# LDeakin/VkVolume

Measured on AMD Instinct MI355X. Metric: Mray/s, higher is better.
Workload: dtype f32

## Files before the change

### vkvolume_amd/csrc/ray_setup.hpp

```cpp
#pragma once

#include "raymarch_args.hpp"
#include "volume_sampling.hpp"

template <int SKIP, bool FAST>
__device__ __forceinline__ bool ray_setup_impl(const RayMarchArgs &A, uint32_t px, uint32_t py, Ray &R, OrdRange &ord)
{
	R.r = R.g = R.b = R.a = 0.0f;
	R.depth = 0.0f;
	R.n_vol = R.n_dist = R.n_empty = 0;
	R.n_steps = 0, R.i = 0, R.i_min = 0, R.first_hit = 0, R.ul = 0;
	R.fragment = false;
	const int W = A.W, H = A.H, D = A.D;

	const float fx = (float) px + 0.5f, fy = (float) py + 0.5f;
	float       dx = __builtin_fmaf(fy, A.ddy[0], __builtin_fmaf(fx, A.ddx[0], A.dir00[0]));
	float       dy = __builtin_fmaf(fy, A.ddy[1], __builtin_fmaf(fx, A.ddx[1], A.dir00[1]));
	float       dz = __builtin_fmaf(fy, A.ddy[2], __builtin_fmaf(fx, A.ddx[2], A.dir00[2]));
	{
		const float len = __builtin_sqrtf(__builtin_fmaf(dz, dz, __builtin_fmaf(dy, dy, dx * dx)));
		if (FAST)
		{
			ord_both(ord, dx, dy, dz);
			const float r = recip_refined(len);
			dx = div_by(dx, len, r), dy = div_by(dy, len, r), dz = div_by(dz, len, r);
		}
		else
			dx /= len, dy /= len, dz /= len;
	}
	const float ox = A.cam[0], oy = A.cam[1], oz = A.cam[2];
	float       t_near = -INFINITY, t_far = INFINITY;
	bool        miss   = false;
	{
		const float dv[3] = {dx, dy, dz}, ov[3] = {ox, oy, oz};
#pragma unroll
		for (int a = 0; a < 3; ++a)
		{
			if (dv[a] == 0.0f)
			{
				if (ov[a] < 0.0f || ov[a] > 1.0f)
					miss = true;
			}
			else
			{
				float inv;
				if (FAST)
				{
					ord_low(ord, dv[a]);
					inv = recip_exact(dv[a]);
				}
				else
					inv = 1.0f / dv[a];
				const float ta = (0.0f - ov[a]) * inv, tb = (1.0f - ov[a]) * inv;
				t_near = g_max(t_near, g_min(ta, tb));
				t_far  = g_min(t_far, g_max(ta, tb));
			}
		}
	}
	if (miss)
		return false;
	const float Ap = __builtin_fmaf(A.plane_tex[2], oz, __builtin_fmaf(A.plane_tex[1], oy, A.plane_tex[0] * ox)) + A.plane_tex[3];
	const float Bp = __builtin_fmaf(A.plane_tex[2], dz, __builtin_fmaf(A.plane_tex[1], dy, A.plane_tex[0] * dx));
	if (!(Bp > 0.0f))
		return false;
	float t_plane;
	if (FAST)
	{
		ord_both(ord, Bp), ord_both(ord, Ap);
		t_plane = div_by(0.0f - Ap, Bp, recip_refined(Bp));
	}
	else
		t_plane = (0.0f - Ap) / Bp;
	const float t0      = g_max(t_near, t_plane);
	if (!(t0 < t_far))
		return false;
	const float ex = __builtin_fmaf(t0, dx, ox), ey = __builtin_fmaf(t0, dy, oy), ez = __builtin_fmaf(t0, dz, oz);
	R.fragment = true;

	float frag_depth = 0.0f, frag_depth_front = 0.0f, position[4] = {0, 0, 0, 0};
	if (A.depth_attachment)
	{
		const float pm[4] = {ex - 0.5f, ey - 0.5f, ez - 0.5f, 1.0f};
		float       a4[4], b4[4];
		mat4_mul_vec4(A.model, pm, a4);
		mat4_mul_vec4(A.view, a4, b4);
		mat4_mul_vec4(A.proj, b4, position);
		frag_depth       = A.in_depth[R.o];
		frag_depth_front = position[2] / position[3];
		if (frag_depth > frag_depth_front)
		{
			R.fragment = false;
			return false;
		}
		R.depth = frag_depth;
	}

	float rdx, rdy, rdz;
	{
		const float vx = ex - ox, vy = ey - oy, vz = ez - oz;
		const float len = __builtin_sqrtf(__builtin_fmaf(vz, vz, __builtin_fmaf(vy, vy, vx * vx)));
		if (FAST)
		{
			ord_both(ord, vx, vy, vz);
			const float r = recip_refined(len);
			rdx = div_by(vx, len, r), rdy = div_by(vy, len, r), rdz = div_by(vz, len, r);
		}
		else
			rdx = vx / len, rdy = vy / len, rdz = vz / len;
	}
	float xx, xy, xz, ray_distance;
	{
		float ix, iy, iz;
		if (FAST)
		{
			ord_low(ord, rdx, rdy, rdz);
			ix = recip_exact(rdx), iy = recip_exact(rdy), iz = recip_exact(rdz);
		}
		else
			ix = 1.0f / rdx, iy = 1.0f / rdy, iz = 1.0f / rdz;
		const float tminx = -ex * ix, tminy = -ey * iy, tminz = -ez * iz;
		const float tmaxx = (1.0f - ex) * ix, tmaxy = (1.0f - ey) * iy, tmaxz = (1.0f - ez) * iz;
		const float t2x = g_max(tminx, tmaxx), t2y = g_max(tminy, tmaxy), t2z = g_max(tminz, tmaxz);
		const float tFar = g_min(g_min(t2x, t2y), t2z);
		xx = __builtin_fmaf(tFar, rdx, ex), xy = __builtin_fmaf(tFar, rdy, ey), xz = __builtin_fmaf(tFar, rdz, ez);
		const float vx = ex - xx, vy = ey - xy, vz = ez - xz;
		ray_distance = __builtin_sqrtf(__builtin_fmaf(vz, vz, __builtin_fmaf(vy, vy, vx * vx)));
	}
	if (A.depth_attachment)
	{
		const float clip[4] = {(position[0] * frag_depth) / frag_depth_front, (position[1] * frag_depth) / frag_depth_front,
		                       (position[2] * frag_depth) / frag_depth_front, position[3]};
		float       w4[4], m4[4];
		mat4_mul_vec4(A.view_proj_inv, clip, w4);
		w4[0] /= w4[3], w4[1] /= w4[3], w4[2] /= w4[3], w4[3] /= w4[3];
		mat4_mul_vec4(A.model_inv, w4, m4);
		const float ix = m4[0] + 0.5f, iy = m4[1] + 0.5f, iz = m4[2] + 0.5f;
		const float vx = ex - ix, vy = ey - iy, vz = ez - iz;
		const float dd = __builtin_sqrtf(__builtin_fmaf(vz, vz, __builtin_fmaf(vy, vy, vx * vx)));
		if (dd < ray_distance)
		{
			xx = ix, xy = iy, xz = iz;
			ray_distance = dd;
		}
	}
	if (A.test == VKV_TEST_RAY_ENTRY)
	{
		R.r = ex, R.g = ey, R.b = ez, R.a = 1.0f;
		return false;
	}
	if (A.test == VKV_TEST_RAY_EXIT)
	{
		R.r = xx, R.g = xy, R.b = xz, R.a = 1.0f;
		return false;
	}

	const int   dim_max = max(max(W, H), D);
	const float nf      = __builtin_ceilf((float) dim_max * ray_distance * A.sampling_factor);
	if (!(nf >= 2.0f && nf <= 16777216.0f))
		return false;
	float sx, sy, sz;
	{
		const float den = nf - 1.0f, nx = rdx * ray_distance, ny = rdy * ray_distance, nz = rdz * ray_distance;
		if (FAST)
		{
			ord_both(ord, nx, ny, nz);
			const float r = recip_refined(den);
			sx = div_by(nx, den, r), sy = div_by(ny, den, r), sz = div_by(nz, den, r);
		}
		else
			sx = nx / den, sy = ny / den, sz = nz / den;
	}
	{
		const float qx = ex + sx, qy = ey + sy, qz = ez + sz;
		if (qx <= 0.0f || qy <= 0.0f || qz <= 0.0f || qx >= 1.0f || qy >= 1.0f || qz >= 1.0f)
			return false;
	}
	R.ex = ex, R.ey = ey, R.ez = ez, R.sx = sx, R.sy = sy, R.sz = sz;
	R.n_steps = (int) nf;

	R.six = R.siy = R.siz = 0.0f;
	R.dmap                = nullptr;
	if (SKIP != VKV_SKIP_NONE)
	{
		if (FAST)
		{
			const float nx = sx * (float) W, ny = sy * (float) H, nz = sz * (float) D;
			ord.lo = ord_min(ord.lo, A.ord_lo0);
			ord_both(ord, nx, ny, nz);
			float tx, ty, tz;
			if (A.block_pow2 != 0u)
				tx = nx * A.block_rcp[0], ty = ny * A.block_rcp[1], tz = nz * A.block_rcp[2];
			else
			{
				tx = div_by(nx, A.block_size[0], recip_refined(A.block_size[0]));
				ty = div_by(ny, A.block_size[1], recip_refined(A.block_size[1]));
				tz = div_by(nz, A.block_size[2], recip_refined(A.block_size[2]));
			}
			ord_both(ord, tx, ty, tz);
			R.six = recip_exact(tx), R.siy = recip_exact(ty), R.siz = recip_exact(tz);
		}
		else
		{
			R.six = 1.0f / ((sx * (float) W) / A.block_size[0]);
			R.siy = 1.0f / ((sy * (float) H) / A.block_size[1]);
			R.siz = 1.0f / ((sz * (float) D) / A.block_size[2]);
		}
		if (SKIP == VKV_SKIP_ANISOTROPIC_DISTANCE)
			R.dmap = A.maps[(rdz < 0 ? 1 : 0) + (rdy < 0 ? 2 : 0) + (rdx < 0 ? 4 : 0)];
		else
			R.dmap = A.maps[0];
	}
	R.i = 0, R.i_min = 0, R.ulx = R.uly = R.ulz = 0, R.ul = 0;
	R.occupied  = true;
	R.first_hit = R.n_steps;
	return true;
}

template <int SKIP>
__device__ __forceinline__ bool ray_setup(const RayMarchArgs &A, uint32_t px, uint32_t py, Ray &R)
{
	OrdRange   ord     = {~0u, 0u};
	const bool marched = ray_setup_impl<SKIP, true>(A, px, py, R, ord);
	if (__builtin_amdgcn_ballot_w64(!ord_ok(ord)) == 0ull)
		return marched;
	OrdRange unused = {~0u, 0u};
	return ray_setup_impl<SKIP, false>(A, px, py, R, unused);
}

__device__ __forceinline__ void ray_clear(Ray &R)
{
	R.r = R.g = R.b = R.a = 0.0f;
	R.depth = 0.0f;
	R.n_vol = R.n_dist = R.n_empty = 0;
	R.n_steps = 0, R.i = 0, R.i_min = 0, R.first_hit = 0, R.ul = 0;
	R.fragment = false;
}

__device__ __forceinline__ void ray_finish(const RayMarchArgs &A, Ray &R, bool marched)
{
	if (marched)
	{
		if (A.out_depth && R.a > 0.0f && R.first_hit < R.n_steps)
		{
			const float fi   = (float) R.first_hit;
			const float p[4] = {__builtin_fmaf(fi, R.sx, R.ex) - 0.5f, __builtin_fmaf(fi, R.sy, R.ey) - 0.5f, __builtin_fmaf(fi, R.sz, R.ez) - 0.5f, 1.0f};
			float       a4[4], b4[4], c4[4];
			mat4_mul_vec4(A.model, p, a4);
			mat4_mul_vec4(A.view, a4, b4);
			mat4_mul_vec4(A.proj, b4, c4);
			R.depth = c4[2] / c4[3];
		}
		if (A.test == VKV_TEST_NUM_TEXTURE_SAMPLES)
		{
			const int      dim_max     = max(max(A.W, A.H), A.D);
			const uint32_t n_steps_max = (uint32_t) (__builtin_ceilf((float) dim_max * __builtin_sqrtf(3.0f)) * A.sampling_factor);
			const float    v           = (float) (R.n_vol + R.n_dist) / (float) n_steps_max;
			R.r = R.g = R.b = v;
			R.a             = 1.0f;
		}
	}
	const size_t o = R.o;
	if (!R.fragment)
	{
		if (A.blend)
		{
			if (A.out_counts)
				A.out_counts[o * 3 + 0] = A.out_counts[o * 3 + 1] = A.out_counts[o * 3 + 2] = 0;
			return;
		}
		if (A.depth_attachment)
			R.depth = A.in_depth[o];
		if (A.out_color)
			store_float4_nt(A.out_color, o, 0.0f, 0.0f, 0.0f, 0.0f);
		if (A.out_rgba8)
			__builtin_nontemporal_store(0u, reinterpret_cast<uint32_t *>(A.out_rgba8) + o);
		if (A.out_counts)
			A.out_counts[o * 3 + 0] = A.out_counts[o * 3 + 1] = A.out_counts[o * 3 + 2] = 0;
		if (A.out_depth)
			__builtin_nontemporal_store(R.depth, A.out_depth + o);
		return;
	}
	else if (A.blend)
	{
		const float om = 1.0f - R.a;
		if (A.out_color)
		{
			float4 d = reinterpret_cast<float4 *>(A.out_color)[o];
			d.x = __builtin_fmaf(om, d.x, R.r), d.y = __builtin_fmaf(om, d.y, R.g), d.z = __builtin_fmaf(om, d.z, R.b), d.w = R.a * om;
			reinterpret_cast<float4 *>(A.out_color)[o] = d;
		}
		if (A.out_rgba8)
		{
			const uint32_t d = reinterpret_cast<uint32_t *>(A.out_rgba8)[o];
			const float    r = __builtin_fmaf(om, unorm8(d & 255u), R.r), g = __builtin_fmaf(om, unorm8((d >> 8) & 255u), R.g),
			            b = __builtin_fmaf(om, unorm8((d >> 16) & 255u), R.b);
			reinterpret_cast<uint32_t *>(A.out_rgba8)[o] = (uint32_t) quantise_rgba8(r) | ((uint32_t) quantise_rgba8(g) << 8) |
			                                               ((uint32_t) quantise_rgba8(b) << 16) | ((uint32_t) quantise_rgba8(R.a * om) << 24);
		}
		if (A.out_counts)
		{
			A.out_counts[o * 3 + 0] = R.n_vol;
			A.out_counts[o * 3 + 1] = R.n_dist;
			A.out_counts[o * 3 + 2] = R.n_empty;
		}
		if (A.out_depth)
			A.out_depth[o] = R.depth;
		return;
	}
	if (A.out_color)
		store_float4_nt(A.out_color, o, R.r, R.g, R.b, R.a);
	if (A.out_rgba8)
		__builtin_nontemporal_store((uint32_t) quantise_rgba8(R.r) | ((uint32_t) quantise_rgba8(R.g) << 8) |
		                                               ((uint32_t) quantise_rgba8(R.b) << 16) | ((uint32_t) quantise_rgba8(R.a) << 24), reinterpret_cast<uint32_t *>(A.out_rgba8) + o);
	if (A.out_counts)
	{
		A.out_counts[o * 3 + 0] = R.n_vol;
		A.out_counts[o * 3 + 1] = R.n_dist;
		A.out_counts[o * 3 + 2] = R.n_empty;
	}
	if (A.out_depth)
		__builtin_nontemporal_store(R.depth, A.out_depth + o);
}

__device__ __forceinline__ uint32_t start_entry(const RayMarchArgs &A, uint32_t r, uint32_t &tx_out, uint32_t &ty_out)
{
	const int w = (int) A.tiles_x, h = (int) A.order_h, rings = (min(w, h) + 1) >> 1;
	auto      inner = [&](int j) { return (w - 2 * j > 0 && h - 2 * j > 0) ? (uint32_t) ((w - 2 * j) * (h - 2 * j)) : 0u; };
	const float d = (float) (w - h);
	int         j = (int) (((float) (w + h) - __builtin_sqrtf(d * d + 4.0f * (float) r)) * 0.25f);
	j             = max(0, min(j, rings - 1));
#pragma unroll
	for (int it = 0; it < 2; ++it)
	{
		if (j + 1 < rings && inner(j + 1) > r)
			++j;
		if (j > 0 && inner(j) <= r)
			--j;
	}
	const int wj = w - 2 * j, hj = h - 2 * j;
	int       q = (int) (r - inner(j + 1)), tx, ty;
	if (hj == 1 || q < wj)
		tx = j + q, ty = j;
	else if ((q -= wj) < hj - 1)
		tx = j + wj - 1, ty = j + 1 + q;
	else if ((q -= hj - 1) < wj - 1)
		tx = j + wj - 2 - q, ty = j + hj - 1;
	else
		q -= wj - 1, tx = j, ty = j + hj - 2 - q;
	tx_out = (uint32_t) __builtin_amdgcn_readfirstlane(tx), ty_out = (uint32_t) __builtin_amdgcn_readfirstlane(ty);
	return ty_out * (uint32_t) w + tx_out;
}
__device__ __forceinline__ uint32_t start_entry(const RayMarchArgs &A, uint32_t r)
{
	uint32_t tx, ty;
	return start_entry(A, r, tx, ty);
}
```

### vkvolume_amd/csrc/raymarch_args.hpp

```cpp
#pragma once

#include <stdint.h>

#include "../host/host_arith.hpp"

constexpr int kTraceWords = 10;
constexpr uint32_t kFillPerTile = 3;

struct RayMarchArgs
{
	float dir00[3], ddx[3], ddy[3];
	float cam[3];
	float plane_tex[4];
	float block_size[3];
	float    block_rcp[3];
	uint32_t block_pow2, ord_lo0;
	float model[16], view[16], proj[16];
	float view_proj_inv[16], model_inv[16];
	float sampling_factor, grad_modifier;
	int W, H, D, mw, mh, md;
	const uint8_t * vol, *grad, *tf;
	const uint8_t * packed;
	int             pmx, pmy;
	const uint32_t *tf_bits;
	const uint8_t * maps[8];
	float *         out_color;
	uint8_t *       out_rgba8;
	uint32_t *      out_counts;
	float *         out_depth;
	const float *   in_depth;
	uint32_t        depth_attachment, blend;
	uint32_t        img_w, img_h, tile_w, tile_h, tiles_x, tile_first, tile_stride, tile_count, compact;
	uint32_t        org_x, org_y;
	uint32_t        fill_tiles, img_tiles_x, rect_tx0, rect_ty0, rect_th;
	uint32_t        fill_rgba8_rows;
	uint32_t        blocks_per_tile_x, blocks_per_tile, nblocks;
	int             test;
	unsigned long long *trace;
	int             back;
	uint32_t        clamp_always;
	float           mapf[3], mapb[3];
	float           cells_per_unit[3], free_margin;
	vkv::UniformDiv div_blocks_per_tile, div_blocks_per_tile_x, div_tiles_x, div_img_tiles_x, div_per_row;
	uint32_t        wave_pw_log2;
	const uint32_t *addr_lut;
	uint32_t        lut_y, lut_z, lut_words;
	uint32_t        lut_full;
	uint32_t        cull_x0, cull_x1, cull_y0, cull_y1;
	const uint32_t *tile_order;
	uint32_t        order_h;
	uint32_t *      queue_heads;
	uint32_t *      tile_cost;
	uint32_t *      order_out;
	float           alpha_lut[256];
};

struct Ray
{
	float          ex, ey, ez;
	float          sx, sy, sz;
	float          six, siy, siz;
	const uint8_t *dmap;
	int            n_steps, i, i_min;
	int            ulx, uly, ulz;
	uint32_t       ul;
	int            first_hit;
	bool           occupied;
	float          r, g, b, a;
	float          depth;
	uint32_t       n_vol, n_dist, n_empty;
	uint32_t       o;
	bool           fragment;
};
```

### vkvolume_amd/csrc/raymarch_core.hpp

```cpp
#pragma once

#include <type_traits>

#include "vkv_device.hpp"
#include "raymarch_args.hpp"
#include "volume_sampling.hpp"
#include "ray_setup.hpp"
#include "raymarch_persistent.hpp"

using namespace vkv;

struct RmLds
{
	union
	{
		struct
		{
			float    alpha[256];
			uint32_t bits[2048];
			float    unorm[256];
		} g;
		struct
		{
			float  ai[258], ag[258];
			float2 pair[256];
		} s;
	};
};

__device__ __forceinline__ bool tf_is_separable(const RayMarchArgs &A)
{
	return A.tf_bits != nullptr && (A.tf_bits[kTfFlagWord] & kTfFlagSeparable) != 0u;
}

__device__ __forceinline__ bool stage_tables_er(const RayMarchArgs &A, RmLds &L, bool sync = true)
{
	const bool sep = tf_is_separable(A);
	typedef const __attribute__((address_space(1))) uint32_t *global_u32_ptr;
	const global_u32_ptr tf_words = (global_u32_ptr) (uintptr_t) A.tf_bits;
	for (int i = threadIdx.x; i < 256; i += blockDim.x)
	{
		const float a = A.alpha_lut[i];
		if (!sep)
			L.g.alpha[i] = a;
		if (sep)
		{
			const float ai = __uint_as_float(tf_words[kTfAiWord + i]), ag = __uint_as_float(tf_words[kTfAgWord + i]);
			L.s.ai[i] = ai, L.s.ag[i] = ag;
			if (i == 255)
				L.s.ai[256] = ai, L.s.ag[256] = ag;
			L.s.pair[i] = i == 0 ? make_float2(0.0f, 0.0f) : make_float2(a, unorm8_staged(i) * a);
		}
		else
			L.g.unorm[i] = unorm8_staged(i);
	}
	if (!sep && A.tf_bits)
		for (int i = threadIdx.x; i < 2048; i += blockDim.x)
			L.g.bits[i] = A.tf_bits[i];
	if (sync)
		__syncthreads();
	return sep;
}
__device__ __forceinline__ void entry_tile(const RayMarchArgs &A, uint32_t k, uint32_t &tx, uint32_t &ty)
{
	uniform_divmod(A.tile_first + k * A.tile_stride, A.tiles_x, A.div_tiles_x, ty, tx);
}
template <int W>
__device__ __forceinline__ bool block_pixel(const RayMarchArgs &A, uint32_t k, uint32_t sbx, uint32_t sby, uint32_t tx, uint32_t ty, uint32_t rb, uint32_t &px, uint32_t &py,
                                            uint32_t &o)
{
	constexpr uint32_t G = 64 / W;
	uint32_t           bx, by;
	const uint32_t     wb = rb / G, g = rb % G;
	if (W == 1)
	{
		const uint32_t pwl = A.wave_pw_log2, pprl = 4u - pwl;
		bx = ((wb & ((1u << pprl) - 1u)) << pwl) + (g & ((1u << pwl) - 1u));
		by = ((wb >> pprl) << (6u - pwl)) + (g >> pwl);
	}
	else
	{
		constexpr uint32_t pw = G >= 32 ? 8 : (G >= 8 ? 4 : 2), ph = G / pw, ppr = 16 / pw;
		bx = (wb % ppr) * pw + g % pw, by = (wb / ppr) * ph + g / pw;
	}
	const uint32_t lx = sbx * 16 + bx, ly = sby * 16 + by;
	px = A.org_x + tx * A.tile_w + lx, py = A.org_y + ty * A.tile_h + ly;
	o  = A.compact ? (k * A.tile_h + ly) * A.tile_w + lx : py * A.img_w + px;
	return px < A.img_w && py < A.img_h;
}
__device__ __forceinline__ int med3_i32(int x, int lo, int hi)
{
	int r;
	asm("v_med3_i32 %0, %1, %2, %3" : "=v"(r) : "v"(x), "v"(lo), "v"(hi));
	return r;
}

template <typename T>
__device__ __forceinline__ T undefined_value()
{
	T x;
	asm volatile("" : "=v"(x));
	return x;
}

__device__ __forceinline__ uint64_t uniform_u64(uint64_t x)
{
	const uint32_t lo = (uint32_t) __builtin_amdgcn_readfirstlane((int) (uint32_t) x), hi = (uint32_t) __builtin_amdgcn_readfirstlane((int) (uint32_t) (x >> 32));
	return ((uint64_t) hi << 32) | lo;
}

__device__ __forceinline__ float uniform_f32(float x)
{
	asm volatile("" : "+v"(x));
	return __builtin_bit_cast(float, __builtin_amdgcn_readfirstlane(__builtin_bit_cast(int, x)));
}

__device__ __forceinline__ float max_f32_raw(float a, float b)
{
	float r;
	asm("v_max_f32 %0, %1, %2" : "=v"(r) : "v"(a), "v"(b));
	return r;
}

__device__ __forceinline__ int clamp0_i32(int x, int hi)
{
	int r;
	asm("v_med3_i32 %0, %1, 0, %2" : "=v"(r) : "v"(x), "s"(hi));
	return r;
}

__device__ __forceinline__ float clamp0_f32_cold(float x, float hi)
{
	float r;
	hi = __builtin_bit_cast(float, __builtin_amdgcn_readfirstlane(__builtin_bit_cast(int, hi)));
	asm volatile("v_med3_f32 %0, %1, 0, %2" : "=v"(r) : "v"(x), "s"(hi));
	return r;
}

__device__ __forceinline__ uint32_t mad_u24(uint32_t a, uint32_t b, uint32_t c)
{
	uint32_t r;
	asm("v_mad_u32_u24 %0, %1, %2, %3" : "=v"(r) : "v"(a), "s"(b), "v"(c));
	return r;
}

constexpr uint32_t kLeanLut      = 1u;
constexpr uint32_t kLeanFull     = 2u;
constexpr uint32_t kLeanNoCounts = 4u;
constexpr uint32_t kLeanSafe     = 16u;
constexpr uint32_t kLeanAsync    = 32u;
constexpr uint32_t kLeanStamp    = 8u;
constexpr size_t   kMaxLutBytes  = 8 * 1024;

__device__ __forceinline__ float cvt_ubyte0(uint32_t q) { float f; asm("v_cvt_f32_ubyte0 %0, %1" : "=v"(f) : "v"(q)); return f; }
__device__ __forceinline__ float cvt_ubyte1(uint32_t q) { float f; asm("v_cvt_f32_ubyte1 %0, %1" : "=v"(f) : "v"(q)); return f; }
__device__ __forceinline__ float cvt_ubyte2(uint32_t q) { float f; asm("v_cvt_f32_ubyte2 %0, %1" : "=v"(f) : "v"(q)); return f; }
__device__ __forceinline__ float cvt_ubyte3(uint32_t q) { float f; asm("v_cvt_f32_ubyte3 %0, %1" : "=v"(f) : "v"(q)); return f; }

template <bool WANT_G, bool TABLE = false>
__device__ __forceinline__ void packed_filter_cvt(uint32_t q00, uint32_t q10, uint32_t q01, uint32_t q11, float wx, float wy, float wz, float &out_v, float &out_g)
{
	constexpr float kScale = TABLE ? kInv255 * 1024.0f : kInv255;
	{
		const float b000 = cvt_ubyte0(q00), b100 = cvt_ubyte2(q00), b010 = cvt_ubyte0(q10), b110 = cvt_ubyte2(q10);
		const float b001 = cvt_ubyte0(q01), b101 = cvt_ubyte2(q01), b011 = cvt_ubyte0(q11), b111 = cvt_ubyte2(q11);
		const float c00 = __builtin_fmaf(wx, b100 - b000, b000), c10 = __builtin_fmaf(wx, b110 - b010, b010);
		const float c01 = __builtin_fmaf(wx, b101 - b001, b001), c11 = __builtin_fmaf(wx, b111 - b011, b011);
		const float c0 = __builtin_fmaf(wy, c10 - c00, c00), c1 = __builtin_fmaf(wy, c11 - c01, c01);
		out_v = __builtin_fmaf(wz, c1 - c0, c0) * kScale;
	}
	if (WANT_G)
	{
		const float b000 = cvt_ubyte1(q00), b100 = cvt_ubyte3(q00), b010 = cvt_ubyte1(q10), b110 = cvt_ubyte3(q10);
		const float b001 = cvt_ubyte1(q01), b101 = cvt_ubyte3(q01), b011 = cvt_ubyte1(q11), b111 = cvt_ubyte3(q11);
		const float c00 = __builtin_fmaf(wx, b100 - b000, b000), c10 = __builtin_fmaf(wx, b110 - b010, b010);
		const float c01 = __builtin_fmaf(wx, b101 - b001, b001), c11 = __builtin_fmaf(wx, b111 - b011, b011);
		const float c0 = __builtin_fmaf(wy, c10 - c00, c00), c1 = __builtin_fmaf(wy, c11 - c01, c01);
		out_g = __builtin_fmaf(wz, c1 - c0, c0) * kScale;
	}
}
extern __shared__ __align__(16) uint32_t s_lean_lds[];
static_assert(sizeof(RmLds) % 16 == 0, "the address tables behind RmLds are read as 64-bit words");

typedef __attribute__((address_space(3))) RmLds *   lds_rmlds_ptr;
typedef __attribute__((address_space(3))) uint32_t *lds_u32_ptr;

constexpr uintptr_t kLdsBase = 16;
__device__ __forceinline__ RmLds &lean_lds() { return *(RmLds *) (lds_rmlds_ptr) kLdsBase; }

__device__ __forceinline__ void lean_lds_check()
{
	uint32_t base = (uint32_t) reinterpret_cast<uintptr_t>(s_lean_lds);
	asm volatile("" : "+s"(base));
	if (base != 0u)
		__builtin_trap();
}

__device__ __forceinline__ bool wg_any(bool pred)
{
	static_assert(kLdsBase >= 16, "the flag words of wg_any sit in front of the tables");
	uint32_t zero = 0u;
	asm volatile("" : "+v"(zero));
	const lds_u32_ptr flags = (lds_u32_ptr) (uintptr_t) zero;
	const bool        mine  = __builtin_amdgcn_ballot_w64(pred) != 0ull;
	if ((threadIdx.x & 63u) == 0u)
		flags[threadIdx.x >> 6] = mine ? 1u : 0u;
	__syncthreads();
	const uint32_t nw  = blockDim.x >> 6;
	typedef uint32_t flags_v4u __attribute__((ext_vector_type(4)));
	const flags_v4u f   = *reinterpret_cast<const __attribute__((address_space(3))) flags_v4u *>(flags);
	const bool      any = (f.x | (nw > 1u ? f.y : 0u) | (nw > 2u ? f.z : 0u) | (nw > 3u ? f.w : 0u)) != 0u;
	return any;
}

#define s_addr_lut ((uint32_t *) (lds_u32_ptr) (kLdsBase + sizeof(RmLds)))
constexpr uint32_t kLutXm = 96;

__device__ __forceinline__ void stage_addr_lut(const RayMarchArgs &A)
{
	for (uint32_t i = threadIdx.x; i < A.lut_z; i += blockDim.x)
		s_addr_lut[i] = A.addr_lut[i];
	const uint64_t base = reinterpret_cast<uint64_t>(A.packed);
	for (uint32_t i = threadIdx.x; 2 * i + A.lut_z < A.lut_words; i += blockDim.x)
	{
		const uint64_t z = (((uint64_t) A.addr_lut[A.lut_z + 2 * i + 1]) << 32 | A.addr_lut[A.lut_z + 2 * i]) + base;
		s_addr_lut[A.lut_z + 2 * i] = (uint32_t) z, s_addr_lut[A.lut_z + 2 * i + 1] = (uint32_t) (z >> 32);
	}
}

template <bool SC = true>
__device__ __forceinline__ const uint8_t *packed_footprint_lut(const RayMarchArgs &A, float px, float py, float pz, float &wx, float &wy, float &wz)
{
	const float cx = __builtin_fmaf(px, (float) A.W, -0.5f), cy = __builtin_fmaf(py, (float) A.H, -0.5f), cz = __builtin_fmaf(pz, (float) A.D, -0.5f);
	const float fx = __builtin_floorf(cx), fy = __builtin_floorf(cy), fz = __builtin_floorf(cz);
	wx = cx - fx, wy = cy - fy, wz = cz - fz;
	const uint32_t tx = (uint32_t) (SC ? clamp0_i32((int) __builtin_fmaf(fx, 4.0f, 4.0f), 4 * (A.W + 1)) : med3_i32((int) __builtin_fmaf(fx, 4.0f, 4.0f), 0, 4 * (A.W + 1)));
	const uint32_t ty = (uint32_t) (SC ? clamp0_i32((int) __builtin_fmaf(fy, 4.0f, 4.0f), 4 * (A.H + 1)) : med3_i32((int) __builtin_fmaf(fy, 4.0f, 4.0f), 0, 4 * (A.H + 1)));
	const uint32_t tz = (uint32_t) (SC ? clamp0_i32((int) __builtin_fmaf(fz, 4.0f, 4.0f), 4 * (A.D + 1)) : med3_i32((int) __builtin_fmaf(fz, 4.0f, 4.0f), 0, 4 * (A.D + 1)));
	const char *   lut = reinterpret_cast<const char *>(s_addr_lut);
	const uint32_t xi = *reinterpret_cast<const uint32_t *>(lut + (tx & 124u)), xm = *reinterpret_cast<const uint32_t *>(lut + 4u * kLutXm + ((tx >> 5) & ~3u));
	const uint32_t yi = *reinterpret_cast<const uint32_t *>(lut + 128u + (ty & 124u)), ym = *reinterpret_cast<const uint32_t *>(lut + 4u * A.lut_y + ((ty >> 5) & ~3u));
	const uint32_t zi = *reinterpret_cast<const uint32_t *>(lut + 256u + (tz & 124u));
	const uint64_t zm = *reinterpret_cast<const uint64_t *>(lut + 4u * A.lut_z + ((tz >> 4) & ~7u));
	return reinterpret_cast<const uint8_t *>(zm + (((xi + xm) + (yi + ym)) + zi));
}

constexpr uint32_t kFullLutWord  = 1028;
__host__ __device__ __forceinline__ bool map_fits_u24(uint32_t mw, uint32_t mh, uint32_t md) { return (uint64_t) mh * md < (1ull << 24) && mw < (1u << 24); }
constexpr size_t   kFullLdsLimit = 17920;

__host__ __device__ __forceinline__ size_t full_lut_bytes(int W, int H, int D) { return (size_t) (W + 2 + H + 2 + D + 2) * 4; }

__host__ __forceinline__ size_t lean_lds_bytes(int kind, uint32_t lut_words, int W, int H, int D)
{
	const size_t two_level = kLdsBase + sizeof(RmLds) + (size_t) lut_words * 4;
	if (kind == 0)
		return kLdsBase + sizeof(RmLds);
	if (kind == 1)
		return two_level;
	const size_t full_end = kLdsBase + (size_t) kFullLutWord * 4 + ((full_lut_bytes(W, H, D) + 15u) & ~(size_t) 15u);
	return two_level > full_end ? two_level : full_end;
}

__device__ __forceinline__ uint32_t *full_lut_base(const RmLds &L) { return const_cast<uint32_t *>(reinterpret_cast<const uint32_t *>(&L)) + kFullLutWord; }

typedef uint32_t lut_v4u __attribute__((ext_vector_type(4)));
constexpr uint32_t kFullCopyRounds = 4;
static_assert((kLdsBase + kFullLutWord * 4) % 16 == 0, "the full tables are written with 16-byte LDS stores");
static_assert(kFullLdsLimit - kFullLutWord * 4 <= kFullCopyRounds * 256 * 16, "the unrolled rounds cover the tables of the default LDS limit");

struct FullLutCopy
{
	lut_v4u  r[kFullCopyRounds];
	uint32_t nvec;
};

__device__ __forceinline__ FullLutCopy full_lut_issue(const RayMarchArgs &A)
{
	typedef const __attribute__((address_space(1))) lut_v4u *global_v4u_ptr;
	FullLutCopy          c;
	const global_v4u_ptr g = (global_v4u_ptr) (uintptr_t) (A.addr_lut + A.lut_full);
	c.nvec                 = ((uint32_t) (A.W + 2 + A.H + 2 + A.D + 2) + 3u) >> 2;
#pragma unroll
	for (uint32_t k = 0; k < kFullCopyRounds; ++k)
		c.r[k] = g[min(threadIdx.x + k * blockDim.x, c.nvec - 1u)];
	return c;
}

__device__ __forceinline__ void full_lut_commit(const RayMarchArgs &A, const FullLutCopy &c, RmLds &L)
{
	static_assert(sizeof(((RmLds *) nullptr)->s) == kFullLutWord * 4, "full tables start behind the separable TF tables");
	typedef const __attribute__((address_space(1))) lut_v4u *global_v4u_ptr;
	lut_v4u *dst = reinterpret_cast<lut_v4u *>(full_lut_base(L));
#pragma unroll
	for (uint32_t k = 0; k < kFullCopyRounds; ++k)
		if (threadIdx.x + k * blockDim.x < c.nvec)
			dst[threadIdx.x + k * blockDim.x] = c.r[k];
	const global_v4u_ptr g = (global_v4u_ptr) (uintptr_t) (A.addr_lut + A.lut_full);
	for (uint32_t i = threadIdx.x + kFullCopyRounds * blockDim.x; i < c.nvec; i += blockDim.x)
		dst[i] = g[i];
}

__device__ __forceinline__ void stage_full_lut(const RayMarchArgs &A, RmLds &L)
{
	const FullLutCopy c = full_lut_issue(A);
	full_lut_commit(A, c, L);
}

struct FullLutConsts
{
	float          w, h, d, oy, oz;
	const uint8_t *base;
};

template <bool SCALAR = false>
__device__ __forceinline__ FullLutConsts full_lut_consts(const RayMarchArgs &A)
{
	FullLutConsts c;
	c.w = (float) A.W, c.h = (float) A.H, c.d = (float) A.D;
	c.base = A.packed;
	c.oy = (float) (4 * (A.W + 2) + 4);
	c.oz = (float) (4 * (A.W + 2 + A.H + 2) + 4);
	if (SCALAR)
		c.w = uniform_f32(c.w), c.h = uniform_f32(c.h), c.d = uniform_f32(c.d), c.oy = uniform_f32(c.oy), c.oz = uniform_f32(c.oz);
	else
		asm volatile("" : "+v"(c.w), "+v"(c.h), "+v"(c.d), "+v"(c.oy), "+v"(c.oz));
	return c;
}

template <bool FREE = false>
__device__ __forceinline__ const uint8_t *packed_footprint_full(const FullLutConsts &C, const RmLds &L, float px, float py, float pz, float &wx, float &wy, float &wz)
{
	const float cx = __builtin_fmaf(px, C.w, -0.5f), cy = __builtin_fmaf(py, C.h, -0.5f), cz = __builtin_fmaf(pz, C.d, -0.5f);
	const float fx = __builtin_floorf(cx), fy = __builtin_floorf(cy), fz = __builtin_floorf(cz);
	wx = cx - fx, wy = cy - fy, wz = cz - fz;
	const int   tx = (int) __builtin_fmaf(FREE ? fx : __builtin_amdgcn_fmed3f(fx, -1.0f, C.w), 4.0f, 4.0f);
	const int   ty = (int) __builtin_fmaf(FREE ? fy : __builtin_amdgcn_fmed3f(fy, -1.0f, C.h), 4.0f, C.oy);
	const int   tz = (int) __builtin_fmaf(FREE ? fz : __builtin_amdgcn_fmed3f(fz, -1.0f, C.d), 4.0f, C.oz);
	const char *   lut = reinterpret_cast<const char *>(full_lut_base(L));
	const uint32_t xo = *reinterpret_cast<const uint32_t *>(lut + tx), yo = *reinterpret_cast<const uint32_t *>(lut + ty);
	const uint32_t zo = *reinterpret_cast<const uint32_t *>(lut + tz);
	return C.base + ((uint64_t) ((xo + yo) + zo) << 1);
}
typedef const __attribute__((address_space(1))) u32_align2 *global_row_ptr;

__device__ __forceinline__ uint32_t load_u8_global(const uint8_t *base, uint32_t index)
{
	typedef const __attribute__((address_space(1))) uint8_t *global_u8_ptr;
	return ((global_u8_ptr) (uintptr_t) base)[index];
}

template <bool NT = false>
__device__ __forceinline__ uint32_t load_row(const uint8_t *p)
{
	global_row_ptr g = (global_row_ptr) (uintptr_t) p;
	if (NT)
		return __builtin_nontemporal_load(g);
	return *g;
}

__device__ __forceinline__ void load_u8_async(uint32_t &dst, const uint8_t *base_uniform, uint32_t index)
{
	asm volatile("global_load_ubyte %0, %1, %2" : "=v"(dst) : "v"(index), "s"(base_uniform));
}
__device__ __forceinline__ void load_u8_async_lane(uint32_t &dst, const uint8_t *base_lane, uint32_t index)
{
	const uint8_t *p = base_lane + index;
	asm volatile("global_load_ubyte %0, %1, off" : "=v"(dst) : "v"(p));
}
__device__ __forceinline__ void load_rows_async(uint32_t &q00, uint32_t &q10, uint32_t &q01, uint32_t &q11, const uint8_t *p)
{
	asm volatile("global_load_dword %0, %4, off\n\tglobal_load_dword %1, %4, off offset:10\n\tglobal_load_dword %2, %4, off offset:50\n\tglobal_load_dword %3, %4, off offset:60"
	             : "=&v"(q00), "=&v"(q10), "=&v"(q01), "=&v"(q11)
	             : "v"(p));
}
__device__ __forceinline__ void wait_oldest_of_five_or_one(uint32_t &a, unsigned long long live)
{
	asm volatile("s_cmp_lg_u64 exec, %1\n\ts_cbranch_scc1 1f\n\ts_waitcnt vmcnt(0)\n\ts_branch 2f\n1:\n\ts_waitcnt vmcnt(4)\n2:" : "+v"(a) : "s"(live) : "scc");
}
__device__ __forceinline__ void wait_rows(uint32_t &q00, uint32_t &q10, uint32_t &q01, uint32_t &q11)
{
	asm volatile("s_waitcnt vmcnt(0)" : "+v"(q00), "+v"(q10), "+v"(q01), "+v"(q11));
}

struct LeanStamp
{
	uint32_t sum[3], cnt[3];
	uint32_t clamped;
};

__device__ __forceinline__ bool lean_safe_at(const RayMarchArgs &A, const Ray &R, float j, float kx, float ky, float kz)
{
	const float px = __builtin_fmaf(j, R.sx, R.ex), py = __builtin_fmaf(j, R.sy, R.ey), pz = __builtin_fmaf(j, R.sz, R.ez);
	const float vx = kx * px, vy = ky * py, vz = kz * pz;
	return __builtin_fminf(__builtin_fminf(vx, vy), vz) >= 0.0f && vx < A.mapf[0] && vy < A.mapf[1] && vz < A.mapf[2];
}

__device__ __forceinline__ bool lean_free_wave(const RayMarchArgs &A, const Ray &R)
{
	if (A.clamp_always)
		return false;
	const float kx = A.cells_per_unit[0], ky = A.cells_per_unit[1], kz = A.cells_per_unit[2];
	const float g  = A.free_margin;
	const float last = (float) R.n_steps - 1.0f;
	const float lx = __builtin_fmaf(last, R.sx, R.ex), ly = __builtin_fmaf(last, R.sy, R.ey), lz = __builtin_fmaf(last, R.sz, R.ez);
	const bool  inside = __builtin_fminf(__builtin_fminf(__builtin_fminf(R.ex, R.ey), R.ez), __builtin_fminf(__builtin_fminf(lx, ly), lz)) >= -g &&
	                    __builtin_fmaxf(__builtin_fmaxf(__builtin_fmaxf(R.ex, R.ey), R.ez), __builtin_fmaxf(__builtin_fmaxf(lx, ly), lz)) <= 1.0f + g;
	const bool free_ray = inside && lean_safe_at(A, R, 1.0f, kx, ky, kz) && (lean_safe_at(A, R, last, kx, ky, kz) || lean_safe_at(A, R, last - 1.0f, kx, ky, kz));
	return __builtin_amdgcn_ballot_w64(!free_ray) == 0ull;
}

template <int SKIP, bool ERT, int GRAD, bool PACKED, bool SEP, uint32_t LF, bool FREE = false>
__device__ __forceinline__ void lean_march(const RayMarchArgs &A, Ray &R, const RmLds &L, uint32_t &iter, LeanStamp &stamp)
{
	constexpr bool kStamp = (LF & kLeanStamp) != 0, kCounts = (LF & kLeanNoCounts) == 0;
	constexpr bool kHoist = PACKED && GRAD != 2;
	constexpr bool kLut = (LF & kLeanLut) != 0, kFull = (LF & kLeanFull) != 0 && SEP, kTf = SEP && kHoist;
	constexpr bool kAsync = (LF & kLeanAsync) != 0 && kTf && SKIP != VKV_SKIP_NONE;
	uint32_t       stamp_prev = 0, stamp_kind = 3;
	const int      W = A.W, H = A.H, D = A.D;
	const float kx = A.cells_per_unit[0], ky = A.cells_per_unit[1], kz = A.cells_per_unit[2];
	if (kLut && !kFull)
	{
		const float fw = (float) W, fh = (float) H, fd = (float) D;
		asm volatile("" : : "v"(fw), "v"(fh), "v"(fd));
	}
	const int   mw1 = A.mw - 1, mh1 = A.mh - 1, md1 = A.md - 1;
	uint32_t amw = (uint32_t) __builtin_amdgcn_readfirstlane(A.mw), amh = (uint32_t) __builtin_amdgcn_readfirstlane(A.mh);
	asm volatile("" : "+s"(amw), "+s"(amh));
	float       grey = 0.0f;
	uint32_t    ul   = 0;
	bool        occ  = true;
	const float sgx = R.six > 0.0f ? 1.0f : -1.0f, sgy = R.siy > 0.0f ? 1.0f : -1.0f, sgz = R.siz > 0.0f ? 1.0f : -1.0f;
	const float ofx = R.six > 0.0f ? 0.0f : 1.0f, ofy = R.siy > 0.0f ? 0.0f : 1.0f, ofz = R.siz > 0.0f ? 0.0f : 1.0f;
	FullLutConsts fullc = {};
	if (kFull)
		fullc = full_lut_consts<FREE>(A);
	float       li = (float) R.i, li_min = (float) R.i_min, lfirst = (float) R.first_hit;
	const float ln = (float) R.n_steps, lback = (float) A.back;
	const uint8_t *const dmap = SKIP == VKV_SKIP_ANISOTROPIC_DISTANCE ? R.dmap : reinterpret_cast<const uint8_t *>(uniform_u64(reinterpret_cast<uintptr_t>(A.maps[0])));
	float lhi_now = -1.0f;
	static_assert(!FREE || ((LF & kLeanSafe) != 0 && kFull && kHoist && SKIP != VKV_SKIP_NONE && !kStamp), "the clamp-free loop exists for kLeanSafe kernels only");
	if (kAsync)
		__builtin_amdgcn_s_waitcnt(0x0F70);
	while (li < ln)
	{
		const float i    = li;
		const float posx = __builtin_fmaf(i, R.sx, R.ex), posy = __builtin_fmaf(i, R.sy, R.ey), posz = __builtin_fmaf(i, R.sz, R.ez);
		int         uix = 0, uiy = 0, uiz = 0;
		float       ux = 0, uy = 0, uz = 0;
		uint32_t    cell = 0;
		if (SKIP != VKV_SKIP_NONE)
		{
			ux = kx * posx, uy = ky * posy, uz = kz * posz;
			if (FREE)
			{
				if (__builtin_expect(__builtin_amdgcn_ballot_w64(i > lhi_now) != 0ull, 0))
				{
					ux = clamp0_f32_cold(ux, A.mapb[0]), uy = clamp0_f32_cold(uy, A.mapb[1]), uz = clamp0_f32_cold(uz, A.mapb[2]);
#ifdef VKV_TRACE_CLAMPED
					++stamp.clamped;
#endif
					float last = ln;
					asm volatile("" : "+v"(last));
					last -= 1.0f;
					lhi_now = lean_safe_at(A, R, last, kx, ky, kz) ? last : last - 1.0f;
				}
				uix = (int) ux, uiy = (int) uy, uiz = (int) uz;
				cell = mad_u24(mad_u24((uint32_t) uiz, amh, (uint32_t) uiy), amw, (uint32_t) uix);
			}
			else if (kLut)
			{
				uix = clamp0_i32((int) ux, mw1), uiy = clamp0_i32((int) uy, mh1), uiz = clamp0_i32((int) uz, md1);
				cell = mad_u24(mad_u24((uint32_t) uiz, amh, (uint32_t) uiy), amw, (uint32_t) uix);
			}
			else
			{
				uix = med3_i32((int) ux, 0, mw1), uiy = med3_i32((int) uy, 0, mh1), uiz = med3_i32((int) uz, 0, md1);
				cell = __umul24(__umul24((uint32_t) uiz, (uint32_t) A.mh) + (uint32_t) uiy, (uint32_t) A.mw) + (uint32_t) uix;
			}
		}
		const bool probe = SKIP != VKV_SKIP_NONE && !occ && cell != ul;
		if (kStamp)
		{
			const uint32_t now = (uint32_t) __builtin_amdgcn_s_memtime();
			const uint32_t dt  = __builtin_amdgcn_readfirstlane(now - stamp_prev);
			if (stamp_kind == 0u)
				stamp.sum[0] = __builtin_amdgcn_readfirstlane(stamp.sum[0] + dt), stamp.cnt[0] = __builtin_amdgcn_readfirstlane(stamp.cnt[0] + 1u);
			else if (stamp_kind == 1u)
				stamp.sum[1] = __builtin_amdgcn_readfirstlane(stamp.sum[1] + dt), stamp.cnt[1] = __builtin_amdgcn_readfirstlane(stamp.cnt[1] + 1u);
			else if (stamp_kind == 2u)
				stamp.sum[2] = __builtin_amdgcn_readfirstlane(stamp.sum[2] + dt), stamp.cnt[2] = __builtin_amdgcn_readfirstlane(stamp.cnt[2] + 1u);
			stamp_prev = now;
			const bool any_p = __builtin_amdgcn_ballot_w64(probe) != 0ull, any_s = __builtin_amdgcn_ballot_w64(!probe) != 0ull;
			stamp_kind       = __builtin_amdgcn_readfirstlane(any_p ? (any_s ? 2u : 0u) : 1u);
		}

		uint32_t dist = undefined_value<uint32_t>(), q00 = undefined_value<uint32_t>(), q10 = undefined_value<uint32_t>(), q01 = undefined_value<uint32_t>(),
		         q11 = undefined_value<uint32_t>();
		float    wx = undefined_value<float>(), wy = undefined_value<float>(), wz = undefined_value<float>();
		unsigned long long live = 0ull;
		if (kAsync)
			live = __builtin_amdgcn_read_exec();
		if (SKIP != VKV_SKIP_NONE && probe)
		{
			if (kAsync && SKIP == VKV_SKIP_ANISOTROPIC_DISTANCE)
				load_u8_async_lane(dist, dmap, cell);
			else if (kAsync)
				load_u8_async(dist, dmap, cell);
			else
				dist = load_u8_global(dmap, cell);
		}
		else if (kHoist)
		{
			const uint8_t *ba = kFull  ? packed_footprint_full<FREE>(fullc, L, posx, posy, posz, wx, wy, wz)
			                    : kLut ? packed_footprint_lut(A, posx, posy, posz, wx, wy, wz)
			                           : packed_footprint(A.packed, W, H, D, A.pmx, A.pmy, posx, posy, posz, wx, wy, wz);
			if (kAsync)
				load_rows_async(q00, q10, q01, q11, ba);
			else
			{
				q00 = load_row(ba);
				q10 = load_row(ba + 10);
				q01 = load_row(ba + 50);
				q11 = load_row(ba + 60);
			}
		}

		float skip = 0.0f;
		auto  probe_outcome = [&]() {
			float bx, by, bz;
			if (SKIP == VKV_SKIP_BLOCK)
				bx = (R.six < 0.0f) ? 0.0f : 1.0f, by = (R.siy < 0.0f) ? 0.0f : 1.0f, bz = (R.siz < 0.0f) ? 0.0f : 1.0f;
			else
			{
				const float fd = (float) dist;
				bx = __builtin_fmaf(sgx, fd, ofx), by = __builtin_fmaf(sgy, fd, ofy), bz = __builtin_fmaf(sgz, fd, ofz);
			}
			float ax, ay, az;
			if (FREE)
			{
				ax = (bx - __builtin_amdgcn_fractf(ux)) * R.six;
				ay = (by - __builtin_amdgcn_fractf(uy)) * R.siy;
				az = (bz - __builtin_amdgcn_fractf(uz)) * R.siz;
			}
			else
			{
				ax = (bx + __builtin_amdgcn_fmed3f((float) uix - ux, -1.0f, 0.0f)) * R.six;
				ay = (by + __builtin_amdgcn_fmed3f((float) uiy - uy, -1.0f, 0.0f)) * R.siy;
				az = (bz + __builtin_amdgcn_fmed3f((float) uiz - uz, -1.0f, 0.0f)) * R.siz;
			}
			const float m = __builtin_fminf(__builtin_fminf(ax, ay), az);
			skip          = __builtin_fmaxf(1.0f, __builtin_ceilf(m));
		};

		float    intensity = 0.0f, gradient = 1.0f;
		uint32_t ab = 0, texel = 0;
		float    a = 0.0f, c = 0.0f;
		auto sample_outcome = [&]() {
			if (kTf)
			{
				const char *ai_tab = reinterpret_cast<const char *>(L.s.ai), *ag_tab = reinterpret_cast<const char *>(L.s.ag);
				float       g_unused;
				if (GRAD == 1)
					packed_filter_cvt<true, true>(q00, q10, q01, q11, wx, wy, wz, intensity, gradient);
				else
					packed_filter_cvt<false, true>(q00, q10, q01, q11, wx, wy, wz, intensity, g_unused);
				const float ai = *reinterpret_cast<const float *>(ai_tab + ((uint32_t) (int) intensity & ~3u));
				float       ag = GRAD == 0 ? L.s.ag[255] : 0.0f;
				if (GRAD == 1)
					ag = *reinterpret_cast<const float *>(ag_tab + ((uint32_t) (int) gradient & ~3u));
				ab              = (uint32_t) ((ai * ag) * 255.0f);
				const float2 pr = L.s.pair[ab];
				a = pr.x, c = pr.y;
				return;
			}
			if (kHoist)
			{
				float unused;
				if (GRAD == 1)
					packed_filter_cvt<true>(q00, q10, q01, q11, wx, wy, wz, intensity, gradient);
				else
					packed_filter_cvt<false>(q00, q10, q01, q11, wx, wy, wz, intensity, unused);
			}
			else if (!probe)
			{
				float unused;
				if (PACKED)
					sample_packed<false>(A.packed, W, H, D, A.pmx, A.pmy, posx, posy, posz, intensity, unused);
				else
				{
					intensity = sample_linear(A.vol, W, H, D, posx, posy, posz);
					if (GRAD == 1)
						gradient = sample_linear(A.grad, W, H, D, posx, posy, posz);
				}
				if (GRAD == 2)
				{
					const float dix = 1.0f / (float) W, diy = 1.0f / (float) H, diz = 1.0f / (float) D;
					float       t1, t2, t3, t4;
					if (PACKED)
					{
						sample_packed<false>(A.packed, W, H, D, A.pmx, A.pmy, posx + dix, posy - diy, posz - diz, t1, unused);
						sample_packed<false>(A.packed, W, H, D, A.pmx, A.pmy, posx - dix, posy - diy, posz + diz, t2, unused);
						sample_packed<false>(A.packed, W, H, D, A.pmx, A.pmy, posx - dix, posy + diy, posz - diz, t3, unused);
						sample_packed<false>(A.packed, W, H, D, A.pmx, A.pmy, posx + dix, posy + diy, posz + diz, t4, unused);
					}
					else
					{
						t1 = sample_linear(A.vol, W, H, D, posx + dix, posy - diy, posz - diz);
						t2 = sample_linear(A.vol, W, H, D, posx - dix, posy - diy, posz + diz);
						t3 = sample_linear(A.vol, W, H, D, posx - dix, posy + diy, posz - diz);
						t4 = sample_linear(A.vol, W, H, D, posx + dix, posy + diy, posz + diz);
					}
					const float gx = (((t1 - t2) - t3) + t4) * 0.25f;
					const float gy = (((-t1 - t2) + t3) + t4) * 0.25f;
					const float gz = (((-t1 + t2) - t3) + t4) * 0.25f;
					const float len = __builtin_sqrtf((gx * gx + gy * gy) + gz * gz);
					gradient = g_clamp(len * A.grad_modifier, 0.0f, 1.0f);
				}
			}
			const uint32_t ti = (uint32_t) min((int) (intensity * 256.0f), 255), tg = GRAD == 0 ? 255u : (uint32_t) min((int) (gradient * 256.0f), 255);
			if (SEP)
			{
				ab              = tf_separable_alpha(L.s.ai[ti], L.s.ag[tg]);
				const float2 pr = L.s.pair[ab];
				a = pr.x, c = pr.y;
			}
			else
			{
				const uint32_t tidx = tg * 256u + ti;
				if (!probe)
				{
					if (A.tf_bits)
					{
						if ((L.g.bits[tidx >> 5] >> (tidx & 31u)) & 1u)
							texel = reinterpret_cast<const uint32_t *>(A.tf)[tidx];
					}
					else
						texel = reinterpret_cast<const uint32_t *>(A.tf)[tidx];
				}
				ab = texel >> 24;
				a  = L.g.alpha[ab];
			}
		};

		__builtin_amdgcn_wave_barrier();
		if (__builtin_expect(probe, 1))
		{
			if (kAsync)
			{
				wait_oldest_of_five_or_one(dist, live);
			}
			probe_outcome();
			if (kCounts)
				++R.n_dist;
			const float back_to = max_f32_raw(i - lback, li_min);
			const bool  hit     = dist == 0u;
			li                  = back_to;
			if (!hit)
				li = i + skip;
			occ  = hit ? true : occ;
			ul   = hit ? cell : ul;
		}
		else
		{
			if (kAsync)
				wait_rows(q00, q10, q01, q11);
			sample_outcome();
			if (kCounts)
				++R.n_vol;
			occ        = ab > 0u;
			bool ended = false;
			const bool blend = kTf ? __builtin_amdgcn_ballot_w64(occ) != 0ull : occ;
			if (blend)
			{
				if (SKIP != VKV_SKIP_NONE)
					ul = (kTf && !occ) ? ul : cell;
				const float om = 1.0f - R.a;
				if (SEP)
					grey = __builtin_fmaf(om, c, grey);
				else
				{
					const float r_ = L.g.unorm[texel & 255u] * a, g_ = L.g.unorm[(texel >> 8) & 255u] * a, b_ = L.g.unorm[(texel >> 16) & 255u] * a;
					R.r = __builtin_fmaf(om, r_, R.r), R.g = __builtin_fmaf(om, g_, R.g), R.b = __builtin_fmaf(om, b_, R.b);
				}
				R.a = __builtin_fmaf(om, a, R.a);
				if (a > 0.0f)
					lfirst = i;
				if (ERT && !kTf)
					ended = R.a > 0.99f;
			}
			if (ERT && kTf)
				ended = R.a > 0.99f;
			if (kCounts && !occ)
				++R.n_empty;
			li_min = i + 1.0f;
			li     = ended ? ln : li_min;
		}
		if (__builtin_amdgcn_readfirstlane(++iter) == 48u)
			__builtin_amdgcn_s_setprio(3);
	}
	if (kStamp)
	{
		const uint32_t dt = (uint32_t) __builtin_amdgcn_s_memtime() - stamp_prev;
		if (stamp_kind == 0u)
			stamp.sum[0] += dt, ++stamp.cnt[0];
		else if (stamp_kind == 1u)
			stamp.sum[1] += dt, ++stamp.cnt[1];
		else if (stamp_kind == 2u)
			stamp.sum[2] += dt, ++stamp.cnt[2];
	}
	R.i = (int) li, R.i_min = (int) li_min, R.first_hit = (int) lfirst;
	if (ERT)
		R.a = R.a > 0.99f ? 1.0f : R.a;
	if (SEP)
		R.r = grey, R.g = grey, R.b = grey;
}

template <int SKIP, bool ERT, int GRAD, bool PACKED, uint32_t LF, int WPB = 4, bool FILL = false>
__device__ __forceinline__ void lean_block(const RayMarchArgs &A, uint32_t bid, RmLds &L)
{
	constexpr uint32_t kParts = 4 / WPB;
	const uint32_t x = bid & 7u, idx = (bid >> 3) / kParts, part = (bid >> 3) % kParts;
	uint32_t group, sb;
	uniform_divmod(idx, A.blocks_per_tile, A.div_blocks_per_tile, group, sb);
	const uint32_t rank = group * 8u + x;
	if (rank >= A.tile_count)
		return;
	const bool computed = !A.tile_order && A.order_h != 0u;
	uint32_t   k = rank, tx = 0, ty = 0;
	if (computed)
		k = start_entry(A, rank, tx, ty);
	else if (A.tile_order)
		k = A.tile_order[rank];
	if (k >= A.tile_count)
		return;
	if (!computed)
		entry_tile(A, k, tx, ty);
	uint32_t sbx, sby;
	uniform_divmod(sb, A.blocks_per_tile_x, A.div_blocks_per_tile_x, sby, sbx);
	const uint32_t lane = threadIdx.x & 63u, wave = threadIdx.x >> 6;
	uint32_t       px, py, o;
	const uint32_t rb = (part * WPB + wave) * 64u + lane;
	if (FILL && A.fill_tiles != 0u)
	{
#pragma unroll
		for (uint32_t it = 0; it < kFillPerTile; ++it)
		{
			const uint32_t j = k + it * A.tile_count;
			if (j >= A.fill_tiles)
				break;
			const uint32_t top = A.rect_ty0 * A.img_tiles_x, per_row = A.img_tiles_x - A.tiles_x, mid = A.rect_th * per_row;
			uint32_t       ftx, fty;
			if (j < top)
				uniform_divmod(j, A.img_tiles_x, A.div_img_tiles_x, fty, ftx);
			else if (j - top < mid)
			{
				uint32_t row, c;
				uniform_divmod(j - top, per_row, A.div_per_row, row, c);
				fty = A.rect_ty0 + row, ftx = c < A.rect_tx0 ? c : c + A.tiles_x;
			}
			else
			{
				uint32_t row;
				uniform_divmod(j - top - mid, A.img_tiles_x, A.div_img_tiles_x, row, ftx);
				fty = A.rect_ty0 + A.rect_th + row;
			}
			const uint32_t bx0 = ftx * A.tile_w + sbx * 16u, by0 = fty * A.tile_h + sby * 16u;
			if (A.fill_rgba8_rows != 0u && bx0 + 16u <= A.img_w)
			{
				if (rb < 64u && by0 + (rb >> 2) < A.img_h)
				{
					typedef uint32_t v4u __attribute__((ext_vector_type(4)));
					const v4u zero = {0u, 0u, 0u, 0u};
					__builtin_nontemporal_store(zero, reinterpret_cast<v4u *>(A.out_rgba8 + ((size_t) (by0 + (rb >> 2)) * A.img_w + bx0 + (rb & 3u) * 4u) * 4u));
				}
			}
			else
			{
				const uint32_t fx = bx0 + (rb & 15u), fy = by0 + (rb >> 4);
				if (fx < A.img_w && fy < A.img_h)
				{
					Ray F;
					ray_clear(F);
					F.o = fy * A.img_w + fx;
					ray_finish(A, F, false);
				}
			}
		}
	}
	const bool     inside = block_pixel<1>(A, k, sbx, sby, tx, ty, rb, px, py, o);
	Ray R;
	R.o = o;
	const unsigned long long t_start = A.trace ? __builtin_amdgcn_s_memrealtime() : 0ull;
	const unsigned long long c_start = A.trace ? __builtin_amdgcn_s_memtime() : 0ull;
	bool marched = false;
	if (inside)
	{
		if (px >= A.cull_x0 && px <= A.cull_x1 && py >= A.cull_y0 && py <= A.cull_y1)
			marched = ray_setup<SKIP>(A, px, py, R);
		else
			ray_clear(R);
	}
	uint32_t  iter  = 0;
	LeanStamp stamp = {};
	if (wg_any(marched))
	{
		bool sep;
		if ((LF & kLeanLut) != 0 && (LF & kLeanFull) != 0 && PACKED && GRAD != 2 && tf_is_separable(A))
		{
			const FullLutCopy c = full_lut_issue(A);
			sep                 = stage_tables_er(A, L, false);
			full_lut_commit(A, c, L);
			__syncthreads();
		}
		else
		{
			if ((LF & kLeanLut) != 0 && PACKED && GRAD != 2)
				stage_addr_lut(A);
			sep = stage_tables_er(A, L);
		}
		if (marched)
		{
			if (sep)
			{
				constexpr bool kSafe = (LF & kLeanSafe) != 0 && (LF & kLeanFull) != 0 && PACKED && GRAD != 2 && SKIP != VKV_SKIP_NONE && (LF & kLeanStamp) == 0;
				if constexpr (kSafe)
				{
					if (lean_free_wave(A, R))
						lean_march<SKIP, ERT, GRAD, PACKED, true, LF, true>(A, R, L, iter, stamp);
					else
						lean_march<SKIP, ERT, GRAD, PACKED, true, LF>(A, R, L, iter, stamp);
				}
				else
					lean_march<SKIP, ERT, GRAD, PACKED, true, LF>(A, R, L, iter, stamp);
			}
			else
				lean_march<SKIP, ERT, GRAD, PACKED, false, LF>(A, R, L, iter, stamp);
		}
	}
	if (A.tile_cost)
	{
		uint32_t it = iter;
		for (int o2 = 32; o2 > 0; o2 >>= 1)
			it = max(it, (uint32_t) __shfl_xor((int) it, o2));
		if (it != 0u && lane == (uint32_t) __builtin_ctzll(__ballot(1)))
			atomicMax(&A.tile_cost[k], it);
	}
	if (!inside)
		return;
	ray_finish(A, R, marched);
	if (A.trace)
	{
		uint32_t it = iter;
		for (int o2 = 32; o2 > 0; o2 >>= 1)
			it = max(it, (uint32_t) __shfl_xor((int) it, o2));
		const unsigned long long t_end = __builtin_amdgcn_s_memrealtime();
		uint32_t clamped_max = stamp.clamped;
		for (int o2 = 32; o2 > 0; o2 >>= 1)
			clamped_max = max(clamped_max, (uint32_t) __shfl_xor((int) clamped_max, o2));
		if ((LF & kLeanStamp) != 0 && iter == it && lane == (uint32_t) __builtin_ctzll(__ballot(iter == it)))
		{
			unsigned long long *rec = A.trace + ((size_t) blockIdx.x * WPB + wave) * kTraceWords;
			rec[4] = ((unsigned long long) stamp.cnt[0] << 32) | stamp.sum[0], rec[5] = ((unsigned long long) stamp.cnt[1] << 32) | stamp.sum[1];
			rec[8] = ((unsigned long long) stamp.cnt[2] << 32) | stamp.sum[2];
		}
		else if ((LF & kLeanStamp) == 0 && lane == (uint32_t) __builtin_ctzll(__ballot(1)))
		{
			unsigned long long *rec = A.trace + ((size_t) blockIdx.x * WPB + wave) * kTraceWords;
			rec[4] = 0, rec[5] = 0, rec[8] = 0;
		}
		if (lane == (uint32_t) __builtin_ctzll(__ballot(1)))
		{
			unsigned long long *rec = A.trace + ((size_t) blockIdx.x * WPB + wave) * kTraceWords;
			rec[0] = t_start, rec[1] = t_end, rec[2] = it, rec[3] = ((unsigned long long) __builtin_amdgcn_s_getreg((3 << 11) | 20) << 32) | (k * A.blocks_per_tile + sb);
			rec[6] = c_start, rec[7] = __builtin_amdgcn_s_memtime(), rec[9] = clamped_max;
		}
	}
}

#if defined(__HIP_DEVICE_COMPILE__) && !defined(VKV_LAB_PACKED_FP32)
#define VKV_NO_PACKED_FP32 __attribute__((target("no-packed-fp32-ops")))
#else
#define VKV_NO_PACKED_FP32
#endif

template <int SKIP, bool ERT, int GRAD, bool PACKED, uint32_t LF>
__global__ void __launch_bounds__(256) k_raymarch_lean(const RayMarchArgs A)
{
	lean_lds_check();
	RmLds &L = lean_lds();
	lean_block<SKIP, ERT, GRAD, PACKED, LF>(A, blockIdx.x, L);
}

template <int SKIP, bool ERT, int GRAD, uint32_t LF>
__global__ void __launch_bounds__(256) VKV_NO_PACKED_FP32 __attribute__((amdgpu_waves_per_eu((GRAD == 2 || SKIP == VKV_SKIP_NONE || (LF & kLeanLut) == 0) ? 1 : 8))) k_raymarch_lean_batch(const RayMarchArgs *__restrict__ frames, uint32_t n, uint32_t groups_per_frame, UniformDiv split)
{
	lean_lds_check();
	RmLds &        L = lean_lds();
	const uint32_t g = blockIdx.x >> 3;
	uint32_t q, r;
	uniform_divmod(g, groups_per_frame == 0 ? n : groups_per_frame, split, q, r);
	const uint32_t f = groups_per_frame == 0 ? r : q, gi = groups_per_frame == 0 ? q : r;
	constexpr uint32_t kLfBatch = (SKIP == VKV_SKIP_ANISOTROPIC_DISTANCE && (LF & kLeanNoCounts) == 0) ? (LF & ~kLeanSafe) : LF;
	lean_block<SKIP, ERT, GRAD, true, kLfBatch, 4, true>(frames[f], (gi << 3) | (blockIdx.x & 7u), L);
}

template <int SKIP, bool ERT, int GRAD, uint32_t LF, bool SEP>
__device__ __forceinline__ void pull_units(const RayMarchArgs *__restrict__ frames, uint32_t n, uint32_t *__restrict__ heads, const RmLds &L)
{
	const RayMarchArgs &A0   = frames[0];
	const uint32_t      lane = threadIdx.x & 63u;
	const uint32_t      upt  = A0.blocks_per_tile * 4u;
	uint32_t            q = blockIdx.x & 7u, open_queues = 0xffu;
	while (open_queues != 0u)
	{
		if (((open_queues >> q) & 1u) == 0u)
		{
			q = (q + 1u) & 7u;
			continue;
		}
		uint32_t v = 0;
		if (lane == 0)
			v = atomicAdd(&heads[q * vkv::kPullHeadStride], 1u);
		v = __builtin_amdgcn_readfirstlane(v);
		const uint32_t tiles_q = A0.tile_count > q ? (A0.tile_count - q + 7u) >> 3 : 0u;
		if (v >= tiles_q * upt * n)
		{
			open_queues &= ~(1u << q);
			q = (q + 1u) & 7u;
			continue;
		}
		const uint32_t      w = v % upt, f = (v / upt) % n, rank = (v / (upt * n)) * 8u + q;
		const RayMarchArgs &A = frames[f];
		const uint32_t      k = A.tile_order ? A.tile_order[rank] : rank;
		if (k >= A.tile_count)
			continue;
		uint32_t            px, py, o;
		uint32_t            tx, ty, sbx, sby;
		entry_tile(A, k, tx, ty);
		uniform_divmod(w >> 2, A.blocks_per_tile_x, A.div_blocks_per_tile_x, sby, sbx);
		const bool          inside = block_pixel<1>(A, k, sbx, sby, tx, ty, (w & 3u) * 64u + lane, px, py, o);
		Ray                 R = {};
		R.o = o;
		const unsigned long long t_start = A.trace ? __builtin_amdgcn_s_memrealtime() : 0ull;
		bool                     marched = false;
		if (inside)
		{
			if (px >= A.cull_x0 && px <= A.cull_x1 && py >= A.cull_y0 && py <= A.cull_y1)
				marched = ray_setup<SKIP>(A, px, py, R);
			else
				ray_clear(R);
		}
		uint32_t                 iter    = 0;
		const unsigned long long t_setup = A.trace ? __builtin_amdgcn_s_memrealtime() : 0ull;
		LeanStamp                unused_stamp = {};
		if (marched)
			lean_march<SKIP, ERT, GRAD, true, SEP, LF>(A, R, L, iter, unused_stamp);
		const unsigned long long t_march = A.trace ? __builtin_amdgcn_s_memrealtime() : 0ull;
		__builtin_amdgcn_s_setprio(0);
		if (A.tile_cost)
		{
			uint32_t it = iter;
			for (int o2 = 32; o2 > 0; o2 >>= 1)
				it = max(it, (uint32_t) __shfl_xor((int) it, o2));
			if (it != 0u && lane == 0u)
				atomicMax(&A.tile_cost[k], it);
		}
		if (inside)
			ray_finish(A, R, marched);
		if (A.trace)
		{
			uint32_t it = iter;
			for (int o2 = 32; o2 > 0; o2 >>= 1)
				it = max(it, (uint32_t) __shfl_xor((int) it, o2));
			const unsigned long long t_end = __builtin_amdgcn_s_memrealtime();
			if (lane == 0)
			{
				unsigned long long *rec = A.trace + ((size_t) ((v / upt) * 8u + q) * upt + w) * kTraceWords;
				rec[0] = t_start, rec[1] = t_end, rec[2] = it, rec[3] = ((unsigned long long) __builtin_amdgcn_s_getreg((3 << 11) | 20) << 32) | (rank * upt + w);
				rec[4] = t_setup, rec[5] = t_march;
				for (int x = 6; x < kTraceWords; ++x)
					rec[x] = 0;
			}
		}
	}
}

template <int SKIP, bool ERT, int GRAD, uint32_t LF>
__global__ void __launch_bounds__(256) __attribute__((amdgpu_waves_per_eu(8, 8))) k_raymarch_lean_pull(const RayMarchArgs *__restrict__ frames, uint32_t n, uint32_t *__restrict__ heads)
{
	lean_lds_check();
	RmLds &             L  = lean_lds();
	const RayMarchArgs &A0 = frames[0];
	bool sep;
	if ((LF & kLeanLut) != 0 && (LF & kLeanFull) != 0 && GRAD != 2 && tf_is_separable(A0))
	{
		const FullLutCopy c = full_lut_issue(A0);
		sep                 = stage_tables_er(A0, L, false);
		full_lut_commit(A0, c, L);
		__syncthreads();
	}
	else
	{
		if ((LF & kLeanLut) != 0 && GRAD != 2)
			stage_addr_lut(A0);
		sep = stage_tables_er(A0, L);
	}
	if (sep)
		pull_units<SKIP, ERT, GRAD, LF, true>(frames, n, heads, L);
	else
		pull_units<SKIP, ERT, GRAD, LF, false>(frames, n, heads, L);
}

namespace vkv
{
int fill_render_args(vkv_ctx *ctx, const VkvRenderParams *P, const float *alpha_lut, RayMarchArgs &a, hipStream_t s, const VkvTuning &T, bool setup, bool batch);
}
```

### vkvolume_amd/csrc/volume_sampling.hpp

```cpp
#pragma once

#include "vkv_device.hpp"

using namespace vkv;

__device__ __forceinline__ float sample_linear(const uint8_t *__restrict__ tex, int W, int H, int D, float px, float py, float pz)
{
	const float cx = __builtin_fmaf(px, (float) W, -0.5f), cy = __builtin_fmaf(py, (float) H, -0.5f), cz = __builtin_fmaf(pz, (float) D, -0.5f);
	const float fx = __builtin_floorf(cx), fy = __builtin_floorf(cy), fz = __builtin_floorf(cz);
	const float wx = cx - fx, wy = cy - fy, wz = cz - fz;
	const int   ix = (int) fx, iy = (int) fy, iz = (int) fz;
	const int   x0 = i_clamp(ix, 0, W - 1), x1 = i_clamp(ix + 1, 0, W - 1);
	const int   y0 = i_clamp(iy, 0, H - 1), y1 = i_clamp(iy + 1, 0, H - 1);
	const int   z0 = i_clamp(iz, 0, D - 1), z1 = i_clamp(iz + 1, 0, D - 1);
	const size_t r00 = ((size_t) z0 * (size_t) H + (size_t) y0) * (size_t) W, r10 = ((size_t) z0 * (size_t) H + (size_t) y1) * (size_t) W;
	const size_t r01 = ((size_t) z1 * (size_t) H + (size_t) y0) * (size_t) W, r11 = ((size_t) z1 * (size_t) H + (size_t) y1) * (size_t) W;
	const float b000 = tex[r00 + x0], b100 = tex[r00 + x1];
	const float b010 = tex[r10 + x0], b110 = tex[r10 + x1];
	const float b001 = tex[r01 + x0], b101 = tex[r01 + x1];
	const float b011 = tex[r11 + x0], b111 = tex[r11 + x1];
	const float c00 = __builtin_fmaf(wx, b100 - b000, b000), c10 = __builtin_fmaf(wx, b110 - b010, b010);
	const float c01 = __builtin_fmaf(wx, b101 - b001, b001), c11 = __builtin_fmaf(wx, b111 - b011, b011);
	const float c0 = __builtin_fmaf(wy, c10 - c00, c00), c1 = __builtin_fmaf(wy, c11 - c01, c01);
	return __builtin_fmaf(wz, c1 - c0, c0) * kInv255;
}

typedef uint32_t u32_align2 __attribute__((aligned(2)));

__device__ __forceinline__ const uint8_t *packed_footprint(const uint8_t *__restrict__ P, int W, int H, int D, int pmx, int pmy, float px, float py, float pz,
                                                           float &wx, float &wy, float &wz)
{
	const float cx = __builtin_fmaf(px, (float) W, -0.5f), cy = __builtin_fmaf(py, (float) H, -0.5f), cz = __builtin_fmaf(pz, (float) D, -0.5f);
	const float fx = __builtin_floorf(cx), fy = __builtin_floorf(cy), fz = __builtin_floorf(cz);
	wx = cx - fx, wy = cy - fy, wz = cz - fz;
	const int bx = i_clamp((int) fx, -1, W) + 1, by = i_clamp((int) fy, -1, H) + 1, bz = i_clamp((int) fz, -1, D) + 1;
	const uint32_t macro = ((uint32_t) (bz >> 5) * (uint32_t) pmy + (uint32_t) (by >> 5)) * (uint32_t) pmx + (uint32_t) (bx >> 5);
	const uint32_t sub   = (uint32_t) ((((bz >> 2) & 7) << 6) | (((by >> 2) & 7) << 3) | ((bx >> 2) & 7));
	const uint32_t in    = (uint32_t) ((((bz & 3) * 5 + (by & 3)) * 5 + (bx & 3)) * 2);
	return P + (((uint64_t) (macro * 512u + sub)) << 8) + in;
}

template <bool WANT_G>
__device__ __forceinline__ void packed_filter(uint32_t q00, uint32_t q10, uint32_t q01, uint32_t q11, float wx, float wy, float wz, float &out_v, float &out_g)
{
	{
		const float b000 = (float) (q00 & 255u), b100 = (float) ((q00 >> 16) & 255u);
		const float b010 = (float) (q10 & 255u), b110 = (float) ((q10 >> 16) & 255u);
		const float b001 = (float) (q01 & 255u), b101 = (float) ((q01 >> 16) & 255u);
		const float b011 = (float) (q11 & 255u), b111 = (float) ((q11 >> 16) & 255u);
		const float c00 = __builtin_fmaf(wx, b100 - b000, b000), c10 = __builtin_fmaf(wx, b110 - b010, b010);
		const float c01 = __builtin_fmaf(wx, b101 - b001, b001), c11 = __builtin_fmaf(wx, b111 - b011, b011);
		const float c0 = __builtin_fmaf(wy, c10 - c00, c00), c1 = __builtin_fmaf(wy, c11 - c01, c01);
		out_v = __builtin_fmaf(wz, c1 - c0, c0) * kInv255;
	}
	if (WANT_G)
	{
		const float b000 = (float) ((q00 >> 8) & 255u), b100 = (float) (q00 >> 24);
		const float b010 = (float) ((q10 >> 8) & 255u), b110 = (float) (q10 >> 24);
		const float b001 = (float) ((q01 >> 8) & 255u), b101 = (float) (q01 >> 24);
		const float b011 = (float) ((q11 >> 8) & 255u), b111 = (float) (q11 >> 24);
		const float c00 = __builtin_fmaf(wx, b100 - b000, b000), c10 = __builtin_fmaf(wx, b110 - b010, b010);
		const float c01 = __builtin_fmaf(wx, b101 - b001, b001), c11 = __builtin_fmaf(wx, b111 - b011, b011);
		const float c0 = __builtin_fmaf(wy, c10 - c00, c00), c1 = __builtin_fmaf(wy, c11 - c01, c01);
		out_g = __builtin_fmaf(wz, c1 - c0, c0) * kInv255;
	}
}

template <bool WANT_G>
__device__ __forceinline__ void sample_packed(const uint8_t *__restrict__ P, int W, int H, int D, int pmx, int pmy, float px, float py, float pz,
                                              float &out_v, float &out_g)
{
	float          wx, wy, wz;
	const uint8_t *b   = packed_footprint(P, W, H, D, pmx, pmy, px, py, pz, wx, wy, wz);
	const uint32_t q00 = *reinterpret_cast<const u32_align2 *>(b);
	const uint32_t q10 = *reinterpret_cast<const u32_align2 *>(b + 10);
	const uint32_t q01 = *reinterpret_cast<const u32_align2 *>(b + 50);
	const uint32_t q11 = *reinterpret_cast<const u32_align2 *>(b + 60);
	packed_filter<WANT_G>(q00, q10, q01, q11, wx, wy, wz, out_v, out_g);
}

__device__ __forceinline__ void mat4_mul_vec4(const float *m, const float *v, float *r)
{
#pragma unroll
	for (int i = 0; i < 4; ++i)
		r[i] = __builtin_fmaf(m[12 + i], v[3], __builtin_fmaf(m[8 + i], v[2], __builtin_fmaf(m[4 + i], v[1], m[i] * v[0])));
}

__device__ __forceinline__ uint8_t quantise_rgba8(float c) { return (uint8_t) __builtin_rintf(g_clamp(c, 0.0f, 1.0f) * 255.0f); }

__device__ __forceinline__ void store_float4_nt(float *base, size_t pixel, float r, float g, float b, float a)
{
	typedef float float4v __attribute__((ext_vector_type(4)));
	const float4v v = {r, g, b, a};
	__builtin_nontemporal_store(v, reinterpret_cast<float4v *>(base) + pixel);
}
```

Baseline: 23010.

## Split kernel args into per-stage structs and use global address-space pointers

```diff
diff --git a/vkvolume_amd/csrc/ray_setup.hpp b/vkvolume_amd/csrc/ray_setup.hpp
--- a/vkvolume_amd/csrc/ray_setup.hpp
+++ b/vkvolume_amd/csrc/ray_setup.hpp
@@ -3,20 +3,19 @@
 #include "raymarch_args.hpp"
 #include "volume_sampling.hpp"
 
-template <int SKIP, bool FAST>
-__device__ __forceinline__ bool ray_setup_impl(const RayMarchArgs &A, uint32_t px, uint32_t py, Ray &R, OrdRange &ord)
+template <int SKIP, bool FAST, bool BATCH = false>
+__device__ __forceinline__ bool ray_setup_impl(const SetupArgs &S, const RayMarchArgs &A, uint32_t px, uint32_t py, Ray &R, OrdRange &ord)
 {
 	R.r = R.g = R.b = R.a = 0.0f;
 	R.depth = 0.0f;
 	R.n_vol = R.n_dist = R.n_empty = 0;
 	R.n_steps = 0, R.i = 0, R.i_min = 0, R.first_hit = 0, R.ul = 0;
 	R.fragment = false;
-	const int W = A.W, H = A.H, D = A.D;
 
 	const float fx = (float) px + 0.5f, fy = (float) py + 0.5f;
-	float       dx = __builtin_fmaf(fy, A.ddy[0], __builtin_fmaf(fx, A.ddx[0], A.dir00[0]));
-	float       dy = __builtin_fmaf(fy, A.ddy[1], __builtin_fmaf(fx, A.ddx[1], A.dir00[1]));
-	float       dz = __builtin_fmaf(fy, A.ddy[2], __builtin_fmaf(fx, A.ddx[2], A.dir00[2]));
+	float       dx = __builtin_fmaf(fy, S.ddy[0], __builtin_fmaf(fx, S.ddx[0], S.dir00[0]));
+	float       dy = __builtin_fmaf(fy, S.ddy[1], __builtin_fmaf(fx, S.ddx[1], S.dir00[1]));
+	float       dz = __builtin_fmaf(fy, S.ddy[2], __builtin_fmaf(fx, S.ddx[2], S.dir00[2]));
 	{
 		const float len = __builtin_sqrtf(__builtin_fmaf(dz, dz, __builtin_fmaf(dy, dy, dx * dx)));
 		if (FAST)
@@ -28,7 +27,7 @@
 		else
 			dx /= len, dy /= len, dz /= len;
 	}
-	const float ox = A.cam[0], oy = A.cam[1], oz = A.cam[2];
+	const float ox = S.cam[0], oy = S.cam[1], oz = S.cam[2];
 	float       t_near = -INFINITY, t_far = INFINITY;
 	bool        miss   = false;
 	{
@@ -59,8 +58,8 @@
 	}
 	if (miss)
 		return false;
-	const float Ap = __builtin_fmaf(A.plane_tex[2], oz, __builtin_fmaf(A.plane_tex[1], oy, A.plane_tex[0] * ox)) + A.plane_tex[3];
-	const float Bp = __builtin_fmaf(A.plane_tex[2], dz, __builtin_fmaf(A.plane_tex[1], dy, A.plane_tex[0] * dx));
+	const float Ap = __builtin_fmaf(S.plane_tex[2], oz, __builtin_fmaf(S.plane_tex[1], oy, S.plane_tex[0] * ox)) + S.plane_tex[3];
+	const float Bp = __builtin_fmaf(S.plane_tex[2], dz, __builtin_fmaf(S.plane_tex[1], dy, S.plane_tex[0] * dx));
 	if (!(Bp > 0.0f))
 		return false;
 	float t_plane;
@@ -78,14 +77,14 @@
 	R.fragment = true;
 
 	float frag_depth = 0.0f, frag_depth_front = 0.0f, position[4] = {0, 0, 0, 0};
-	if (A.depth_attachment)
+	if (S.depth_attachment)
 	{
 		const float pm[4] = {ex - 0.5f, ey - 0.5f, ez - 0.5f, 1.0f};
 		float       a4[4], b4[4];
 		mat4_mul_vec4(A.model, pm, a4);
 		mat4_mul_vec4(A.view, a4, b4);
 		mat4_mul_vec4(A.proj, b4, position);
-		frag_depth       = A.in_depth[R.o];
+		frag_depth       = as_global(A.in_depth)[R.o];
 		frag_depth_front = position[2] / position[3];
 		if (frag_depth > frag_depth_front)
 		{
@@ -126,7 +125,7 @@
 		const float vx = ex - xx, vy = ey - xy, vz = ez - xz;
 		ray_distance = __builtin_sqrtf(__builtin_fmaf(vz, vz, __builtin_fmaf(vy, vy, vx * vx)));
 	}
-	if (A.depth_attachment)
+	if (S.depth_attachment)
 	{
 		const float clip[4] = {(position[0] * frag_depth) / frag_depth_front, (position[1] * frag_depth) / frag_depth_front,
 		                       (position[2] * frag_depth) / frag_depth_front, position[3]};
@@ -143,19 +142,22 @@
 			ray_distance = dd;
 		}
 	}
-	if (A.test == VKV_TEST_RAY_ENTRY)
+	const SetupStepArgs  step_copy = BATCH ? static_cast<const SetupStepArgs &>(A) : SetupStepArgs{};
+	const SetupStepArgs &T         = BATCH ? step_copy : static_cast<const SetupStepArgs &>(A);
+	const int            W = T.W, H = T.H, D = T.D;
+	if (T.test == VKV_TEST_RAY_ENTRY)
 	{
 		R.r = ex, R.g = ey, R.b = ez, R.a = 1.0f;
 		return false;
 	}
-	if (A.test == VKV_TEST_RAY_EXIT)
+	if (T.test == VKV_TEST_RAY_EXIT)
 	{
 		R.r = xx, R.g = xy, R.b = xz, R.a = 1.0f;
 		return false;
 	}
 
 	const int   dim_max = max(max(W, H), D);
-	const float nf      = __builtin_ceilf((float) dim_max * ray_distance * A.sampling_factor);
+	const float nf      = __builtin_ceilf((float) dim_max * ray_distance * T.sampling_factor);
 	if (!(nf >= 2.0f && nf <= 16777216.0f))
 		return false;
 	float sx, sy, sz;
@@ -185,25 +187,25 @@
 		if (FAST)
 		{
 			const float nx = sx * (float) W, ny = sy * (float) H, nz = sz * (float) D;
-			ord.lo = ord_min(ord.lo, A.ord_lo0);
+			ord.lo = ord_min(ord.lo, T.ord_lo0);
 			ord_both(ord, nx, ny, nz);
 			float tx, ty, tz;
-			if (A.block_pow2 != 0u)
-				tx = nx * A.block_rcp[0], ty = ny * A.block_rcp[1], tz = nz * A.block_rcp[2];
+			if (T.block_pow2 != 0u)
+				tx = nx * T.block_rcp[0], ty = ny * T.block_rcp[1], tz = nz * T.block_rcp[2];
 			else
 			{
-				tx = div_by(nx, A.block_size[0], recip_refined(A.block_size[0]));
-				ty = div_by(ny, A.block_size[1], recip_refined(A.block_size[1]));
-				tz = div_by(nz, A.block_size[2], recip_refined(A.block_size[2]));
+				tx = div_by(nx, T.block_size[0], recip_refined(T.block_size[0]));
+				ty = div_by(ny, T.block_size[1], recip_refined(T.block_size[1]));
+				tz = div_by(nz, T.block_size[2], recip_refined(T.block_size[2]));
 			}
 			ord_both(ord, tx, ty, tz);
 			R.six = recip_exact(tx), R.siy = recip_exact(ty), R.siz = recip_exact(tz);
 		}
 		else
 		{
-			R.six = 1.0f / ((sx * (float) W) / A.block_size[0]);
-			R.siy = 1.0f / ((sy * (float) H) / A.block_size[1]);
-			R.siz = 1.0f / ((sz * (float) D) / A.block_size[2]);
+			R.six = 1.0f / ((sx * (float) W) / T.block_size[0]);
+			R.siy = 1.0f / ((sy * (float) H) / T.block_size[1]);
+			R.siz = 1.0f / ((sz * (float) D) / T.block_size[2]);
 		}
 		if (SKIP == VKV_SKIP_ANISOTROPIC_DISTANCE)
 			R.dmap = A.maps[(rdz < 0 ? 1 : 0) + (rdy < 0 ? 2 : 0) + (rdx < 0 ? 4 : 0)];
@@ -216,15 +218,20 @@
 	return true;
 }
 
-template <int SKIP>
-__device__ __forceinline__ bool ray_setup(const RayMarchArgs &A, uint32_t px, uint32_t py, Ray &R)
+template <int SKIP, bool BATCH = true>
+__device__ __forceinline__ bool ray_setup(const SetupArgs &S, const RayMarchArgs &A, uint32_t px, uint32_t py, Ray &R)
 {
 	OrdRange   ord     = {~0u, 0u};
-	const bool marched = ray_setup_impl<SKIP, true>(A, px, py, R, ord);
+	const bool marched = ray_setup_impl<SKIP, true, BATCH>(S, A, px, py, R, ord);
 	if (__builtin_amdgcn_ballot_w64(!ord_ok(ord)) == 0ull)
 		return marched;
 	OrdRange unused = {~0u, 0u};
-	return ray_setup_impl<SKIP, false>(A, px, py, R, unused);
+	return ray_setup_impl<SKIP, false, BATCH>(S, A, px, py, R, unused);
+}
+template <int SKIP>
+__device__ __forceinline__ bool ray_setup(const RayMarchArgs &A, uint32_t px, uint32_t py, Ray &R)
+{
+	return ray_setup<SKIP, false>(A, A, px, py, R);
 }
 
 __device__ __forceinline__ void ray_clear(Ray &R)
@@ -236,11 +243,14 @@
 	R.fragment = false;
 }
 
-__device__ __forceinline__ void ray_finish(const RayMarchArgs &A, Ray &R, bool marched)
-{
+template <class Finish>
+__device__ __forceinline__ void ray_finish(const Finish &F, const RayMarchArgs &A, Ray &R, bool marched)
+{
+	const auto out_color = as_global(F.out_color), out_depth = as_global(F.out_depth);
+	const auto out_rgba8 = as_global(reinterpret_cast<uint32_t *>(F.out_rgba8)), out_counts = as_global(F.out_counts);
 	if (marched)
 	{
-		if (A.out_depth && R.a > 0.0f && R.first_hit < R.n_steps)
+		if (out_depth && R.a > 0.0f && R.first_hit < R.n_steps)
 		{
 			const float fi   = (float) R.first_hit;
 			const float p[4] = {__builtin_fmaf(fi, R.sx, R.ex) - 0.5f, __builtin_fmaf(fi, R.sy, R.ey) - 0.5f, __builtin_fmaf(fi, R.sz, R.ez) - 0.5f, 1.0f};
@@ -250,7 +260,7 @@
 			mat4_mul_vec4(A.proj, b4, c4);
 			R.depth = c4[2] / c4[3];
 		}
-		if (A.test == VKV_TEST_NUM_TEXTURE_SAMPLES)
+		if (F.test == VKV_TEST_NUM_TEXTURE_SAMPLES)
 		{
 			const int      dim_max     = max(max(A.W, A.H), A.D);
 			const uint32_t n_steps_max = (uint32_t) (__builtin_ceilf((float) dim_max * __builtin_sqrtf(3.0f)) * A.sampling_factor);
@@ -262,67 +272,72 @@
 	const size_t o = R.o;
 	if (!R.fragment)
 	{
-		if (A.blend)
-		{
-			if (A.out_counts)
-				A.out_counts[o * 3 + 0] = A.out_counts[o * 3 + 1] = A.out_counts[o * 3 + 2] = 0;
+		if (F.blend)
+		{
+			if (out_counts)
+				out_counts[o * 3 + 0] = out_counts[o * 3 + 1] = out_counts[o * 3 + 2] = 0;
 			return;
 		}
-		if (A.depth_attachment)
-			R.depth = A.in_depth[o];
-		if (A.out_color)
-			store_float4_nt(A.out_color, o, 0.0f, 0.0f, 0.0f, 0.0f);
-		if (A.out_rgba8)
-			__builtin_nontemporal_store(0u, reinterpret_cast<uint32_t *>(A.out_rgba8) + o);
-		if (A.out_counts)
-			A.out_counts[o * 3 + 0] = A.out_counts[o * 3 + 1] = A.out_counts[o * 3 + 2] = 0;
-		if (A.out_depth)
-			__builtin_nontemporal_store(R.depth, A.out_depth + o);
+		if (F.depth_attachment)
+			R.depth = as_global(A.in_depth)[o];
+		if (out_color)
+			store_float4_nt(out_color, o, 0.0f, 0.0f, 0.0f, 0.0f);
+		if (out_rgba8)
+			__builtin_nontemporal_store(0u, out_rgba8 + o);
+		if (out_counts)
+			out_counts[o * 3 + 0] = out_counts[o * 3 + 1] = out_counts[o * 3 + 2] = 0;
+		if (out_depth)
+			__builtin_nontemporal_store(R.depth, out_depth + o);
 		return;
 	}
-	else if (A.blend)
+	else if (F.blend)
 	{
 		const float om = 1.0f - R.a;
-		if (A.out_color)
-		{
-			float4 d = reinterpret_cast<float4 *>(A.out_color)[o];
+		if (out_color)
+		{
+			typedef float float4v __attribute__((ext_vector_type(4)));
+			float4v       d = reinterpret_cast<global_ptr<float4v>>(out_color)[o];
 			d.x = __builtin_fmaf(om, d.x, R.r), d.y = __builtin_fmaf(om, d.y, R.g), d.z = __builtin_fmaf(om, d.z, R.b), d.w = R.a * om;
-			reinterpret_cast<float4 *>(A.out_color)[o] = d;
-		}
-		if (A.out_rgba8)
-		{
-			const uint32_t d = reinterpret_cast<uint32_t *>(A.out_rgba8)[o];
+			reinterpret_cast<global_ptr<float4v>>(out_color)[o] = d;
+		}
+		if (out_rgba8)
+		{
+			const uint32_t d = out_rgba8[o];
 			const float    r = __builtin_fmaf(om, unorm8(d & 255u), R.r), g = __builtin_fmaf(om, unorm8((d >> 8) & 255u), R.g),
 			            b = __builtin_fmaf(om, unorm8((d >> 16) & 255u), R.b);
-			reinterpret_cast<uint32_t *>(A.out_rgba8)[o] = (uint32_t) quantise_rgba8(r) | ((uint32_t) quantise_rgba8(g) << 8) |
+			out_rgba8[o] = (uint32_t) quantise_rgba8(r) | ((uint32_t) quantise_rgba8(g) << 8) |
 			                                               ((uint32_t) quantise_rgba8(b) << 16) | ((uint32_t) quantise_rgba8(R.a * om) << 24);
 		}
-		if (A.out_counts)
-		{
-			A.out_counts[o * 3 + 0] = R.n_vol;
-			A.out_counts[o * 3 + 1] = R.n_dist;
-			A.out_counts[o * 3 + 2] = R.n_empty;
-		}
-		if (A.out_depth)
-			A.out_depth[o] = R.depth;
+		if (out_counts)
+		{
+			out_counts[o * 3 + 0] = R.n_vol;
+			out_counts[o * 3 + 1] = R.n_dist;
+			out_counts[o * 3 + 2] = R.n_empty;
+		}
+		if (out_depth)
+			out_depth[o] = R.depth;
 		return;
 	}
-	if (A.out_color)
-		store_float4_nt(A.out_color, o, R.r, R.g, R.b, R.a);
-	if (A.out_rgba8)
+	if (out_color)
+		store_float4_nt(out_color, o, R.r, R.g, R.b, R.a);
+	if (out_rgba8)
 		__builtin_nontemporal_store((uint32_t) quantise_rgba8(R.r) | ((uint32_t) quantise_rgba8(R.g) << 8) |
-		                                               ((uint32_t) quantise_rgba8(R.b) << 16) | ((uint32_t) quantise_rgba8(R.a) << 24), reinterpret_cast<uint32_t *>(A.out_rgba8) + o);
-	if (A.out_counts)
-	{
-		A.out_counts[o * 3 + 0] = R.n_vol;
-		A.out_counts[o * 3 + 1] = R.n_dist;
-		A.out_counts[o * 3 + 2] = R.n_empty;
-	}
-	if (A.out_depth)
-		__builtin_nontemporal_store(R.depth, A.out_depth + o);
-}
-
-__device__ __forceinline__ uint32_t start_entry(const RayMarchArgs &A, uint32_t r, uint32_t &tx_out, uint32_t &ty_out)
+		                                               ((uint32_t) quantise_rgba8(R.b) << 16) | ((uint32_t) quantise_rgba8(R.a) << 24), out_rgba8 + o);
+	if (out_counts)
+	{
+		out_counts[o * 3 + 0] = R.n_vol;
+		out_counts[o * 3 + 1] = R.n_dist;
+		out_counts[o * 3 + 2] = R.n_empty;
+	}
+	if (out_depth)
+		__builtin_nontemporal_store(R.depth, out_depth + o);
+}
+__device__ __forceinline__ void ray_finish(const RayMarchArgs &A, Ray &R, bool marched)
+{
+	ray_finish(A, A, R, marched);
+}
+
+__device__ __forceinline__ uint32_t start_entry(const DealArgs &A, uint32_t r, uint32_t &tx_out, uint32_t &ty_out)
 {
 	const int w = (int) A.tiles_x, h = (int) A.order_h, rings = (min(w, h) + 1) >> 1;
 	auto      inner = [&](int j) { return (w - 2 * j > 0 && h - 2 * j > 0) ? (uint32_t) ((w - 2 * j) * (h - 2 * j)) : 0u; };
@@ -350,7 +365,7 @@
 	tx_out = (uint32_t) __builtin_amdgcn_readfirstlane(tx), ty_out = (uint32_t) __builtin_amdgcn_readfirstlane(ty);
 	return ty_out * (uint32_t) w + tx_out;
 }
-__device__ __forceinline__ uint32_t start_entry(const RayMarchArgs &A, uint32_t r)
+__device__ __forceinline__ uint32_t start_entry(const DealArgs &A, uint32_t r)
 {
 	uint32_t tx, ty;
 	return start_entry(A, r, tx, ty);
diff --git a/vkvolume_amd/csrc/raymarch_args.hpp b/vkvolume_amd/csrc/raymarch_args.hpp
--- a/vkvolume_amd/csrc/raymarch_args.hpp
+++ b/vkvolume_amd/csrc/raymarch_args.hpp
@@ -7,52 +7,83 @@
 constexpr int kTraceWords = 10;
 constexpr uint32_t kFillPerTile = 3;
 
-struct RayMarchArgs
+
+struct alignas(16) DealArgs
+{
+	uint32_t        blocks_per_tile_x, blocks_per_tile, nblocks, tile_count;
+	vkv::UniformDiv div_blocks_per_tile, div_blocks_per_tile_x, div_tiles_x, div_img_tiles_x, div_per_row;
+	uint32_t        tiles_x, order_h;
+	const uint32_t *tile_order;
+	uint32_t        tile_first, tile_stride, compact, wave_pw_log2;
+	uint32_t        img_w, img_h, tile_w, tile_h;
+	uint32_t        org_x, org_y;
+	uint32_t        fill_tiles, img_tiles_x, rect_tx0, rect_ty0, rect_th;
+	uint32_t        fill_rgba8_rows;
+	uint32_t        cull_x0, cull_x1, cull_y0, cull_y1;
+};
+
+struct alignas(16) SetupArgs
 {
 	float dir00[3], ddx[3], ddy[3];
 	float cam[3];
 	float plane_tex[4];
-	float block_size[3];
+	uint32_t depth_attachment;
+};
+
+struct alignas(16) SetupStepArgs
+{
+	int      test;
+	int W, H, D;
+	float sampling_factor, grad_modifier;
 	float    block_rcp[3];
 	uint32_t block_pow2, ord_lo0;
+	float    block_size[3];
+};
+
+struct alignas(16) DepthArgs
+{
 	float model[16], view[16], proj[16];
 	float view_proj_inv[16], model_inv[16];
-	float sampling_factor, grad_modifier;
-	int W, H, D, mw, mh, md;
+	const float *in_depth;
+};
+
+struct alignas(16) StageArgs
+{
+	const uint32_t *tf_bits;
+	const uint32_t *addr_lut;
+	uint32_t        lut_y, lut_z, lut_words;
+	uint32_t        lut_full;
 	const uint8_t * vol, *grad, *tf;
+	int             pmx, pmy;
+};
+
+struct alignas(16) MarchArgs
+{
 	const uint8_t * packed;
-	int             pmx, pmy;
-	const uint32_t *tf_bits;
 	const uint8_t * maps[8];
+	float           cells_per_unit[3], free_margin;
+	int             mw, mh, md;
+	int             back;
+	float           mapf[3], mapb[3];
+	uint32_t        clamp_always;
+};
+
+struct alignas(16) FinishArgs
+{
 	float *         out_color;
 	uint8_t *       out_rgba8;
 	uint32_t *      out_counts;
 	float *         out_depth;
-	const float *   in_depth;
-	uint32_t        depth_attachment, blend;
-	uint32_t        img_w, img_h, tile_w, tile_h, tiles_x, tile_first, tile_stride, tile_count, compact;
-	uint32_t        org_x, org_y;
-	uint32_t        fill_tiles, img_tiles_x, rect_tx0, rect_ty0, rect_th;
-	uint32_t        fill_rgba8_rows;
-	uint32_t        blocks_per_tile_x, blocks_per_tile, nblocks;
-	int             test;
+	uint32_t *      tile_cost;
 	unsigned long long *trace;
-	int             back;
-	uint32_t        clamp_always;
-	float           mapf[3], mapb[3];
-	float           cells_per_unit[3], free_margin;
-	vkv::UniformDiv div_blocks_per_tile, div_blocks_per_tile_x, div_tiles_x, div_img_tiles_x, div_per_row;
-	uint32_t        wave_pw_log2;
-	const uint32_t *addr_lut;
-	uint32_t        lut_y, lut_z, lut_words;
-	uint32_t        lut_full;
-	uint32_t        cull_x0, cull_x1, cull_y0, cull_y1;
-	const uint32_t *tile_order;
-	uint32_t        order_h;
+	uint32_t *      order_out;
 	uint32_t *      queue_heads;
-	uint32_t *      tile_cost;
-	uint32_t *      order_out;
-	float           alpha_lut[256];
+	uint32_t        blend;
+};
+
+struct RayMarchArgs : DealArgs, SetupArgs, SetupStepArgs, DepthArgs, StageArgs, MarchArgs, FinishArgs
+{
+	float alpha_lut[256];
 };
 
 struct Ray
diff --git a/vkvolume_amd/csrc/raymarch_core.hpp b/vkvolume_amd/csrc/raymarch_core.hpp
--- a/vkvolume_amd/csrc/raymarch_core.hpp
+++ b/vkvolume_amd/csrc/raymarch_core.hpp
@@ -30,7 +30,7 @@
 
 __device__ __forceinline__ bool tf_is_separable(const RayMarchArgs &A)
 {
-	return A.tf_bits != nullptr && (A.tf_bits[kTfFlagWord] & kTfFlagSeparable) != 0u;
+	return A.tf_bits != nullptr && (as_global(A.tf_bits)[kTfFlagWord] & kTfFlagSeparable) != 0u;
 }
 
 __device__ __forceinline__ bool stage_tables_er(const RayMarchArgs &A, RmLds &L, bool sync = true)
@@ -56,17 +56,17 @@
 	}
 	if (!sep && A.tf_bits)
 		for (int i = threadIdx.x; i < 2048; i += blockDim.x)
-			L.g.bits[i] = A.tf_bits[i];
+			L.g.bits[i] = tf_words[i];
 	if (sync)
 		__syncthreads();
 	return sep;
 }
-__device__ __forceinline__ void entry_tile(const RayMarchArgs &A, uint32_t k, uint32_t &tx, uint32_t &ty)
+__device__ __forceinline__ void entry_tile(const DealArgs &A, uint32_t k, uint32_t &tx, uint32_t &ty)
 {
 	uniform_divmod(A.tile_first + k * A.tile_stride, A.tiles_x, A.div_tiles_x, ty, tx);
 }
 template <int W>
-__device__ __forceinline__ bool block_pixel(const RayMarchArgs &A, uint32_t k, uint32_t sbx, uint32_t sby, uint32_t tx, uint32_t ty, uint32_t rb, uint32_t &px, uint32_t &py,
+__device__ __forceinline__ bool block_pixel(const DealArgs &A, uint32_t k, uint32_t sbx, uint32_t sby, uint32_t tx, uint32_t ty, uint32_t rb, uint32_t &px, uint32_t &py,
                                             uint32_t &o)
 {
 	constexpr uint32_t G = 64 / W;
@@ -313,8 +313,8 @@
 	const uint8_t *base;
 };
 
-template <bool SCALAR = false>
-__device__ __forceinline__ FullLutConsts full_lut_consts(const RayMarchArgs &A)
+template <bool SCALAR = false, class Args>
+__device__ __forceinline__ FullLutConsts full_lut_consts(const Args &A)
 {
 	FullLutConsts c;
 	c.w = (float) A.W, c.h = (float) A.H, c.d = (float) A.D;
@@ -389,14 +389,16 @@
 	uint32_t clamped;
 };
 
-__device__ __forceinline__ bool lean_safe_at(const RayMarchArgs &A, const Ray &R, float j, float kx, float ky, float kz)
+template <class Args>
+__device__ __forceinline__ bool lean_safe_at(const Args &A, const Ray &R, float j, float kx, float ky, float kz)
 {
 	const float px = __builtin_fmaf(j, R.sx, R.ex), py = __builtin_fmaf(j, R.sy, R.ey), pz = __builtin_fmaf(j, R.sz, R.ez);
 	const float vx = kx * px, vy = ky * py, vz = kz * pz;
 	return __builtin_fminf(__builtin_fminf(vx, vy), vz) >= 0.0f && vx < A.mapf[0] && vy < A.mapf[1] && vz < A.mapf[2];
 }
 
-__device__ __forceinline__ bool lean_free_wave(const RayMarchArgs &A, const Ray &R)
+template <class Args>
+__device__ __forceinline__ bool lean_free_wave(const Args &A, const Ray &R)
 {
 	if (A.clamp_always)
 		return false;
@@ -410,23 +412,23 @@
 	return __builtin_amdgcn_ballot_w64(!free_ray) == 0ull;
 }
 
-template <int SKIP, bool ERT, int GRAD, bool PACKED, bool SEP, uint32_t LF, bool FREE = false>
-__device__ __forceinline__ void lean_march(const RayMarchArgs &A, Ray &R, const RmLds &L, uint32_t &iter, LeanStamp &stamp)
+template <int SKIP, bool ERT, int GRAD, bool PACKED, bool SEP, uint32_t LF, bool FREE = false, class Head>
+__device__ __forceinline__ void lean_march(const Head &M, const RayMarchArgs &A, Ray &R, const RmLds &L, uint32_t &iter, LeanStamp &stamp)
 {
 	constexpr bool kStamp = (LF & kLeanStamp) != 0, kCounts = (LF & kLeanNoCounts) == 0;
 	constexpr bool kHoist = PACKED && GRAD != 2;
 	constexpr bool kLut = (LF & kLeanLut) != 0, kFull = (LF & kLeanFull) != 0 && SEP, kTf = SEP && kHoist;
 	constexpr bool kAsync = (LF & kLeanAsync) != 0 && kTf && SKIP != VKV_SKIP_NONE;
 	uint32_t       stamp_prev = 0, stamp_kind = 3;
-	const int      W = A.W, H = A.H, D = A.D;
-	const float kx = A.cells_per_unit[0], ky = A.cells_per_unit[1], kz = A.cells_per_unit[2];
+	const int      W = M.W, H = M.H, D = M.D;
+	const float kx = M.cells_per_unit[0], ky = M.cells_per_unit[1], kz = M.cells_per_unit[2];
 	if (kLut && !kFull)
 	{
 		const float fw = (float) W, fh = (float) H, fd = (float) D;
 		asm volatile("" : : "v"(fw), "v"(fh), "v"(fd));
 	}
-	const int   mw1 = A.mw - 1, mh1 = A.mh - 1, md1 = A.md - 1;
-	uint32_t amw = (uint32_t) __builtin_amdgcn_readfirstlane(A.mw), amh = (uint32_t) __builtin_amdgcn_readfirstlane(A.mh);
+	const int   mw1 = M.mw - 1, mh1 = M.mh - 1, md1 = M.md - 1;
+	uint32_t amw = (uint32_t) __builtin_amdgcn_readfirstlane(M.mw), amh = (uint32_t) __builtin_amdgcn_readfirstlane(M.mh);
 	asm volatile("" : "+s"(amw), "+s"(amh));
 	float       grey = 0.0f;
 	uint32_t    ul   = 0;
@@ -435,10 +437,10 @@
 	const float ofx = R.six > 0.0f ? 0.0f : 1.0f, ofy = R.siy > 0.0f ? 0.0f : 1.0f, ofz = R.siz > 0.0f ? 0.0f : 1.0f;
 	FullLutConsts fullc = {};
 	if (kFull)
-		fullc = full_lut_consts<FREE>(A);
+		fullc = full_lut_consts<FREE>(M);
 	float       li = (float) R.i, li_min = (float) R.i_min, lfirst = (float) R.first_hit;
-	const float ln = (float) R.n_steps, lback = (float) A.back;
-	const uint8_t *const dmap = SKIP == VKV_SKIP_ANISOTROPIC_DISTANCE ? R.dmap : reinterpret_cast<const uint8_t *>(uniform_u64(reinterpret_cast<uintptr_t>(A.maps[0])));
+	const float ln = (float) R.n_steps, lback = (float) M.back;
+	const uint8_t *const dmap = SKIP == VKV_SKIP_ANISOTROPIC_DISTANCE ? R.dmap : reinterpret_cast<const uint8_t *>(uniform_u64(reinterpret_cast<uintptr_t>(M.maps[0])));
 	float lhi_now = -1.0f;
 	static_assert(!FREE || ((LF & kLeanSafe) != 0 && kFull && kHoist && SKIP != VKV_SKIP_NONE && !kStamp), "the clamp-free loop exists for kLeanSafe kernels only");
 	if (kAsync)
@@ -717,79 +719,88 @@
 		R.r = grey, R.g = grey, R.b = grey;
 }
 
+template <int SKIP, bool ERT, int GRAD, bool PACKED, bool SEP, uint32_t LF, bool FREE = false>
+__device__ __forceinline__ void lean_march(const RayMarchArgs &A, Ray &R, const RmLds &L, uint32_t &iter, LeanStamp &stamp)
+{
+	lean_march<SKIP, ERT, GRAD, PACKED, SEP, LF, FREE>(A, A, R, L, iter, stamp);
+}
+
 template <int SKIP, bool ERT, int GRAD, bool PACKED, uint32_t LF, int WPB = 4, bool FILL = false>
 __device__ __forceinline__ void lean_block(const RayMarchArgs &A, uint32_t bid, RmLds &L)
 {
 	constexpr uint32_t kParts = 4 / WPB;
+	const DealArgs  deal  = A;
+	uint8_t *const  fill_rgba8 = A.out_rgba8;
 	const uint32_t x = bid & 7u, idx = (bid >> 3) / kParts, part = (bid >> 3) % kParts;
 	uint32_t group, sb;
-	uniform_divmod(idx, A.blocks_per_tile, A.div_blocks_per_tile, group, sb);
+	uniform_divmod(idx, deal.blocks_per_tile, deal.div_blocks_per_tile, group, sb);
 	const uint32_t rank = group * 8u + x;
-	if (rank >= A.tile_count)
+	if (rank >= deal.tile_count)
 		return;
-	const bool computed = !A.tile_order && A.order_h != 0u;
+	const bool computed = !deal.tile_order && deal.order_h != 0u;
 	uint32_t   k = rank, tx = 0, ty = 0;
 	if (computed)
-		k = start_entry(A, rank, tx, ty);
-	else if (A.tile_order)
-		k = A.tile_order[rank];
-	if (k >= A.tile_count)
+		k = start_entry(deal, rank, tx, ty);
+	else if (deal.tile_order)
+		k = as_global(deal.tile_order)[rank];
+	if (k >= deal.tile_count)
 		return;
 	if (!computed)
-		entry_tile(A, k, tx, ty);
+		entry_tile(deal, k, tx, ty);
 	uint32_t sbx, sby;
-	uniform_divmod(sb, A.blocks_per_tile_x, A.div_blocks_per_tile_x, sby, sbx);
+	uniform_divmod(sb, deal.blocks_per_tile_x, deal.div_blocks_per_tile_x, sby, sbx);
 	const uint32_t lane = threadIdx.x & 63u, wave = threadIdx.x >> 6;
 	uint32_t       px, py, o;
 	const uint32_t rb = (part * WPB + wave) * 64u + lane;
-	if (FILL && A.fill_tiles != 0u)
+	if (FILL && deal.fill_tiles != 0u)
 	{
 #pragma unroll
 		for (uint32_t it = 0; it < kFillPerTile; ++it)
 		{
-			const uint32_t j = k + it * A.tile_count;
-			if (j >= A.fill_tiles)
+			const uint32_t j = k + it * deal.tile_count;
+			if (j >= deal.fill_tiles)
 				break;
-			const uint32_t top = A.rect_ty0 * A.img_tiles_x, per_row = A.img_tiles_x - A.tiles_x, mid = A.rect_th * per_row;
+			const uint32_t top = deal.rect_ty0 * deal.img_tiles_x, per_row = deal.img_tiles_x - deal.tiles_x, mid = deal.rect_th * per_row;
 			uint32_t       ftx, fty;
 			if (j < top)
-				uniform_divmod(j, A.img_tiles_x, A.div_img_tiles_x, fty, ftx);
+				uniform_divmod(j, deal.img_tiles_x, deal.div_img_tiles_x, fty, ftx);
 			else if (j - top < mid)
 			{
 				uint32_t row, c;
-				uniform_divmod(j - top, per_row, A.div_per_row, row, c);
-				fty = A.rect_ty0 + row, ftx = c < A.rect_tx0 ? c : c + A.tiles_x;
+				uniform_divmod(j - top, per_row, deal.div_per_row, row, c);
+				fty = deal.rect_ty0 + row, ftx = c < deal.rect_tx0 ? c : c + deal.tiles_x;
 			}
 			else
 			{
 				uint32_t row;
-				uniform_divmod(j - top - mid, A.img_tiles_x, A.div_img_tiles_x, row, ftx);
-				fty = A.rect_ty0 + A.rect_th + row;
-			}
-			const uint32_t bx0 = ftx * A.tile_w + sbx * 16u, by0 = fty * A.tile_h + sby * 16u;
-			if (A.fill_rgba8_rows != 0u && bx0 + 16u <= A.img_w)
-			{
-				if (rb < 64u && by0 + (rb >> 2) < A.img_h)
+				uniform_divmod(j - top - mid, deal.img_tiles_x, deal.div_img_tiles_x, row, ftx);
+				fty = deal.rect_ty0 + deal.rect_th + row;
+			}
+			const uint32_t bx0 = ftx * deal.tile_w + sbx * 16u, by0 = fty * deal.tile_h + sby * 16u;
+			if (deal.fill_rgba8_rows != 0u && bx0 + 16u <= deal.img_w)
+			{
+				if (rb < 64u && by0 + (rb >> 2) < deal.img_h)
 				{
 					typedef uint32_t v4u __attribute__((ext_vector_type(4)));
 					const v4u zero = {0u, 0u, 0u, 0u};
-					__builtin_nontemporal_store(zero, reinterpret_cast<v4u *>(A.out_rgba8 + ((size_t) (by0 + (rb >> 2)) * A.img_w + bx0 + (rb & 3u) * 4u) * 4u));
+					__builtin_nontemporal_store(zero, as_global(reinterpret_cast<v4u *>(fill_rgba8 + ((size_t) (by0 + (rb >> 2)) * deal.img_w + bx0 + (rb & 3u) * 4u) * 4u)));
 				}
 			}
 			else
 			{
 				const uint32_t fx = bx0 + (rb & 15u), fy = by0 + (rb >> 4);
-				if (fx < A.img_w && fy < A.img_h)
+				if (fx < deal.img_w && fy < deal.img_h)
 				{
 					Ray F;
 					ray_clear(F);
-					F.o = fy * A.img_w + fx;
+					F.o = fy * deal.img_w + fx;
 					ray_finish(A, F, false);
 				}
 			}
 		}
 	}
-	const bool     inside = block_pixel<1>(A, k, sbx, sby, tx, ty, rb, px, py, o);
+	const SetupArgs setup = A;
+	const bool     inside = block_pixel<1>(deal, k, sbx, sby, tx, ty, rb, px, py, o);
 	Ray R;
 	R.o = o;
 	const unsigned long long t_start = A.trace ? __builtin_amdgcn_s_memrealtime() : 0ull;
@@ -797,8 +808,8 @@
 	bool marched = false;
 	if (inside)
 	{
-		if (px >= A.cull_x0 && px <= A.cull_x1 && py >= A.cull_y0 && py <= A.cull_y1)
-			marched = ray_setup<SKIP>(A, px, py, R);
+		if (px >= deal.cull_x0 && px <= deal.cull_x1 && py >= deal.cull_y0 && py <= deal.cull_y1)
+			marched = ray_setup<SKIP>(setup, A, px, py, R);
 		else
 			ray_clear(R);
 	}
@@ -806,6 +817,18 @@
 	LeanStamp stamp = {};
 	if (wg_any(marched))
 	{
+		struct MarchHead : MarchArgs
+		{
+			int W, H, D;
+		};
+		MarchHead march = {static_cast<const MarchArgs &>(A), A.W, A.H, A.D};
+		if constexpr (FILL)
+		{
+			uint32_t off = (uint32_t) (reinterpret_cast<const char *>(A.mapf) - reinterpret_cast<const char *>(&A));
+			asm volatile("" : "+s"(off));
+			const float *mapf = reinterpret_cast<const float *>(reinterpret_cast<const char *>(&A) + off);
+			march.mapf[0] = mapf[0], march.mapf[1] = mapf[1], march.mapf[2] = mapf[2];
+		}
 		bool sep;
 		if ((LF & kLeanLut) != 0 && (LF & kLeanFull) != 0 && PACKED && GRAD != 2 && tf_is_separable(A))
 		{
@@ -827,30 +850,36 @@
 				constexpr bool kSafe = (LF & kLeanSafe) != 0 && (LF & kLeanFull) != 0 && PACKED && GRAD != 2 && SKIP != VKV_SKIP_NONE && (LF & kLeanStamp) == 0;
 				if constexpr (kSafe)
 				{
-					if (lean_free_wave(A, R))
-						lean_march<SKIP, ERT, GRAD, PACKED, true, LF, true>(A, R, L, iter, stamp);
+					if (lean_free_wave(march, R))
+						lean_march<SKIP, ERT, GRAD, PACKED, true, LF, true>(march, A, R, L, iter, stamp);
 					else
-						lean_march<SKIP, ERT, GRAD, PACKED, true, LF>(A, R, L, iter, stamp);
+						lean_march<SKIP, ERT, GRAD, PACKED, true, LF>(march, A, R, L, iter, stamp);
 				}
 				else
-					lean_march<SKIP, ERT, GRAD, PACKED, true, LF>(A, R, L, iter, stamp);
+					lean_march<SKIP, ERT, GRAD, PACKED, true, LF>(march, A, R, L, iter, stamp);
 			}
 			else
-				lean_march<SKIP, ERT, GRAD, PACKED, false, LF>(A, R, L, iter, stamp);
-		}
-	}
-	if (A.tile_cost)
+				lean_march<SKIP, ERT, GRAD, PACKED, false, LF>(march, A, R, L, iter, stamp);
+		}
+	}
+	struct Finish : FinishArgs
+	{
+		uint32_t depth_attachment;
+		int      test;
+	};
+	const Finish fin = {static_cast<const FinishArgs &>(A), A.depth_attachment, A.test};
+	if (fin.tile_cost)
 	{
 		uint32_t it = iter;
 		for (int o2 = 32; o2 > 0; o2 >>= 1)
 			it = max(it, (uint32_t) __shfl_xor((int) it, o2));
 		if (it != 0u && lane == (uint32_t) __builtin_ctzll(__ballot(1)))
-			atomicMax(&A.tile_cost[k], it);
+			__hip_atomic_fetch_max(as_global(fin.tile_cost) + k, it, __ATOMIC_RELAXED, __HIP_MEMORY_SCOPE_AGENT);
 	}
 	if (!inside)
 		return;
-	ray_finish(A, R, marched);
-	if (A.trace)
+	ray_finish(fin, A, R, marched);
+	if (fin.trace)
 	{
 		uint32_t it = iter;
 		for (int o2 = 32; o2 > 0; o2 >>= 1)
@@ -861,18 +890,18 @@
 			clamped_max = max(clamped_max, (uint32_t) __shfl_xor((int) clamped_max, o2));
 		if ((LF & kLeanStamp) != 0 && iter == it && lane == (uint32_t) __builtin_ctzll(__ballot(iter == it)))
 		{
-			unsigned long long *rec = A.trace + ((size_t) blockIdx.x * WPB + wave) * kTraceWords;
+			const auto rec = as_global(fin.trace) + ((size_t) blockIdx.x * WPB + wave) * kTraceWords;
 			rec[4] = ((unsigned long long) stamp.cnt[0] << 32) | stamp.sum[0], rec[5] = ((unsigned long long) stamp.cnt[1] << 32) | stamp.sum[1];
 			rec[8] = ((unsigned long long) stamp.cnt[2] << 32) | stamp.sum[2];
 		}
 		else if ((LF & kLeanStamp) == 0 && lane == (uint32_t) __builtin_ctzll(__ballot(1)))
 		{
-			unsigned long long *rec = A.trace + ((size_t) blockIdx.x * WPB + wave) * kTraceWords;
+			const auto rec = as_global(fin.trace) + ((size_t) blockIdx.x * WPB + wave) * kTraceWords;
 			rec[4] = 0, rec[5] = 0, rec[8] = 0;
 		}
 		if (lane == (uint32_t) __builtin_ctzll(__ballot(1)))
 		{
-			unsigned long long *rec = A.trace + ((size_t) blockIdx.x * WPB + wave) * kTraceWords;
+			const auto rec = as_global(fin.trace) + ((size_t) blockIdx.x * WPB + wave) * kTraceWords;
 			rec[0] = t_start, rec[1] = t_end, rec[2] = it, rec[3] = ((unsigned long long) __builtin_amdgcn_s_getreg((3 << 11) | 20) << 32) | (k * A.blocks_per_tile + sb);
 			rec[6] = c_start, rec[7] = __builtin_amdgcn_s_memtime(), rec[9] = clamped_max;
 		}
diff --git a/vkvolume_amd/csrc/volume_sampling.hpp b/vkvolume_amd/csrc/volume_sampling.hpp
--- a/vkvolume_amd/csrc/volume_sampling.hpp
+++ b/vkvolume_amd/csrc/volume_sampling.hpp
@@ -88,6 +88,19 @@
 
 __device__ __forceinline__ uint8_t quantise_rgba8(float c) { return (uint8_t) __builtin_rintf(g_clamp(c, 0.0f, 1.0f) * 255.0f); }
 
+template <class T>
+using global_ptr = __attribute__((address_space(1))) T *;
+template <class T>
+__device__ __forceinline__ global_ptr<T> as_global(T *p)
+{
+	return (global_ptr<T>) (uintptr_t) p;
+}
+__device__ __forceinline__ void store_float4_nt(global_ptr<float> base, size_t pixel, float r, float g, float b, float a)
+{
+	typedef float float4v __attribute__((ext_vector_type(4)));
+	const float4v v = {r, g, b, a};
+	__builtin_nontemporal_store(v, reinterpret_cast<global_ptr<float4v>>(base) + pixel);
+}
 __device__ __forceinline__ void store_float4_nt(float *base, size_t pixel, float r, float g, float b, float a)
 {
 	typedef float float4v __attribute__((ext_vector_type(4)));
```

Result: no change. 23160, median of 2 (+0.7%).
